# facebookresearch/vggsfm

Measured on NVIDIA H100. Metric: BA iterations/sec, higher is better.
Workload: dtype f64

## Files before the change

vggsfm_b200/_lib.py:

```python
from __future__ import annotations

import ctypes
import os

_HERE = os.path.dirname(os.path.abspath(__file__))
LIB_PATH = os.path.join(_HERE, "libvggsfm_b200.so")

EXPORTS = [
    "vgg_last_error", "vgg_version",
    "vgg_ba_default_options", "vgg_ba_dims", "vgg_ba_workspace_bytes", "vgg_ba_camrec_len",
    "vgg_ba_build_blocks", "vgg_ba_schur", "vgg_cholesky_lower", "vgg_ba_solve",
    "vgg_ba_reduced_system_doubles", "vgg_ba_fabric_doubles", "vgg_ba_solve_fabric",
    "vgg_pose_default_options", "vgg_pose_refinement", "vgg_pnp_workspace_bytes", "vgg_absolute_pose_estimation", "vgg_syrk_ozaki_workspace_bytes", "vgg_syrk_ozaki",
    "vgg_tri_workspace_bytes", "vgg_triangulate_tracks", "vgg_triangulate_by_pair", "vgg_filter_points3d",
    "vgg_project_points", "vgg_normalize_tracks", "vgg_undistort_simple_radial",
    "vgg_corr_pyramid_bytes", "vgg_corr_build_pyramid", "vgg_corr_sample", "vgg_sample_features4d",
    "vgg_corr_tc_supported", "vgg_corr_tc_bytes", "vgg_corr_tc_build", "vgg_corr_tc_sample",
    "vgg_twoview_workspace_bytes", "vgg_estimate_fundamental", "vgg_relative_pose_from_fundamental",
    "vgg_fundamental_inliers", "vgg_msac_fundamental_workspace_bytes", "vgg_estimate_fundamental_msac",
    "vgg_depth_sparse_samples", "vgg_depth_median", "vgg_depth_ransac_workspace_bytes", "vgg_depth_ransac_max_chunk",
    "vgg_depth_ransac_begin", "vgg_depth_ransac_chunk", "vgg_depth_ransac_finish", "vgg_depth_tile_pixels",
    "vgg_depth_apply", "vgg_depth_unproject",
]


DEV_EXPORTS = ["vgg_dev_blocks_timing", "vgg_dev_blocks_last_ms", "vgg_dev_chol128_probe", "vgg_dev_syrk_f64", "vgg_dev_syrk_f64_band", "vgg_dev_syrk_ozaki_band", "vgg_dev_trsv_probe", "vgg_dev_cholesky_band",
               "vgg_dev_last_band_hint", "vgg_dev_msac_trace"]


class BAProblem(ctypes.Structure):
    _fields_ = [
        ("S", ctypes.c_int32), ("N", ctypes.c_int32),
        ("camera_model", ctypes.c_int32), ("intr_mode", ctypes.c_int32),
        ("uv", ctypes.c_void_p), ("mask", ctypes.c_void_p),
        ("param_const", ctypes.c_void_p), ("point_const", ctypes.c_void_p),
        ("poses", ctypes.c_void_p), ("intr", ctypes.c_void_p), ("points", ctypes.c_void_p),
    ]


class BAOptions(ctypes.Structure):
    _fields_ = [
        ("max_num_iterations", ctypes.c_int32),
        ("max_num_consecutive_invalid_steps", ctypes.c_int32),
        ("jacobi_scaling", ctypes.c_int32),
        ("reserved", ctypes.c_int32),
        ("function_tolerance", ctypes.c_double),
        ("gradient_tolerance", ctypes.c_double),
        ("parameter_tolerance", ctypes.c_double),
        ("initial_trust_region_radius", ctypes.c_double),
        ("max_trust_region_radius", ctypes.c_double),
        ("min_trust_region_radius", ctypes.c_double),
        ("min_relative_decrease", ctypes.c_double),
        ("min_lm_diagonal", ctypes.c_double),
        ("max_lm_diagonal", ctypes.c_double),
    ]


class BASummary(ctypes.Structure):
    _fields_ = [
        ("iterations", ctypes.c_int32), ("successful", ctypes.c_int32),
        ("termination", ctypes.c_int32), ("reserved", ctypes.c_int32),
        ("initial_cost", ctypes.c_double), ("final_cost", ctypes.c_double),
        ("final_radius", ctypes.c_double), ("device_ms", ctypes.c_double),
        ("kernel_launches", ctypes.c_int64),
    ]


class BAFabric(ctypes.Structure):
    _fields_ = [("ar_local", ctypes.c_void_p), ("ar_multicast", ctypes.c_void_p), ("ar_doubles", ctypes.c_size_t),
                ("world", ctypes.c_int32), ("rank", ctypes.c_int32), ("peer_base", ctypes.c_void_p * 8),
                ("total_doubles", ctypes.c_size_t)]


class PoseOptions(ctypes.Structure):
    _fields_ = [
        ("max_num_iterations", ctypes.c_int32),
        ("max_num_consecutive_invalid_steps", ctypes.c_int32),
        ("min_inliers", ctypes.c_int32),
        ("reserved", ctypes.c_int32),
        ("function_tolerance", ctypes.c_double),
        ("gradient_tolerance", ctypes.c_double),
        ("parameter_tolerance", ctypes.c_double),
        ("initial_trust_region_radius", ctypes.c_double),
        ("max_trust_region_radius", ctypes.c_double),
        ("min_trust_region_radius", ctypes.c_double),
        ("min_relative_decrease", ctypes.c_double),
        ("min_lm_diagonal", ctypes.c_double),
        ("max_lm_diagonal", ctypes.c_double),
        ("loss_function_scale", ctypes.c_double),
        ("max_reproj_error", ctypes.c_double),
    ]


ALLREDUCE_FN = ctypes.CFUNCTYPE(ctypes.c_int, ctypes.c_void_p, ctypes.c_void_p, ctypes.c_size_t,
                                ctypes.c_int, ctypes.c_void_p)

_lib = None


class NativeLibraryMissing(RuntimeError):
    pass


def lib() -> ctypes.CDLL:
    global _lib
    if _lib is not None:
        return _lib
    if not os.path.exists(LIB_PATH):
        raise NativeLibraryMissing(
            f"{LIB_PATH} not found: build it with `python -c 'import __graft_entry__ as g; g.build()'` "
            "or `make`. vggsfm_b200 has no CPU/PyTorch fallback.")
    L = ctypes.CDLL(LIB_PATH, mode=ctypes.RTLD_GLOBAL)
    L.vgg_last_error.restype = ctypes.c_char_p
    L.vgg_version.restype = ctypes.c_int
    L.vgg_ba_default_options.argtypes = [ctypes.POINTER(BAOptions)]
    L.vgg_ba_default_options.restype = None
    L.vgg_ba_dims.argtypes = [ctypes.c_int, ctypes.c_int, ctypes.POINTER(ctypes.c_int), ctypes.POINTER(ctypes.c_int)]
    L.vgg_ba_workspace_bytes.argtypes = [ctypes.c_int, ctypes.c_int, ctypes.c_int, ctypes.c_int,
                                         ctypes.POINTER(ctypes.c_size_t)]
    L.vgg_ba_camrec_len.argtypes = [ctypes.c_int, ctypes.c_int]
    L.vgg_ba_build_blocks.argtypes = [ctypes.POINTER(BAProblem)] + [ctypes.c_void_p] * 6 + [ctypes.c_int, ctypes.c_void_p]
    L.vgg_ba_schur.argtypes = ([ctypes.POINTER(BAProblem)] + [ctypes.c_void_p] * 6 +
                               [ctypes.c_double] * 3 + [ctypes.c_void_p, ctypes.c_size_t, ctypes.c_void_p,
                                                        ctypes.c_void_p, ctypes.POINTER(ctypes.c_int), ctypes.c_void_p])
    L.vgg_ba_solve.argtypes = [ctypes.POINTER(BAProblem), ctypes.POINTER(BAOptions), ctypes.c_void_p, ctypes.c_size_t,
                               ALLREDUCE_FN, ctypes.c_void_p, ctypes.POINTER(BASummary), ctypes.c_void_p,
                               ctypes.c_void_p]
    vp, ci, cd, cs = ctypes.c_void_p, ctypes.c_int, ctypes.c_double, ctypes.c_size_t
    L.vgg_ba_reduced_system_doubles.argtypes = [ci, ci, ci, ctypes.POINTER(cs)]
    L.vgg_ba_fabric_doubles.argtypes = [ci, ci, ci, ctypes.POINTER(cs)]
    L.vgg_ba_solve_fabric.argtypes = [ctypes.POINTER(BAProblem), ctypes.POINTER(BAOptions), vp, cs, ALLREDUCE_FN, vp,
                                      ctypes.POINTER(BAFabric), ctypes.POINTER(BASummary), vp, vp]
    L.vgg_pose_default_options.argtypes = [ctypes.POINTER(PoseOptions)]
    L.vgg_pose_default_options.restype = None
    L.vgg_pose_refinement.argtypes = [ci, ci, ci, vp, vp, vp, vp, vp, vp, ctypes.POINTER(PoseOptions), vp, vp, vp, vp]
    L.vgg_pnp_workspace_bytes.argtypes = [ci, ci, ctypes.POINTER(cs)]
    L.vgg_absolute_pose_estimation.argtypes = [ci, ci, ci, vp, vp, vp, vp, vp, vp, ci, ci, cd, vp, vp, vp, vp, vp, cs, vp]
    L.vgg_syrk_ozaki_workspace_bytes.argtypes = [ci, ci, ci, ctypes.POINTER(cs)]
    L.vgg_dev_blocks_timing.argtypes = [ci]
    L.vgg_dev_blocks_last_ms.argtypes = [ctypes.POINTER(cd)]
    L.vgg_dev_chol128_probe.argtypes = [ci, vp, vp, vp]
    L.vgg_dev_syrk_f64.argtypes = [ci, ci, vp, vp, vp]
    L.vgg_dev_syrk_f64_band.argtypes = L.vgg_dev_syrk_f64.argtypes + [vp, ci]
    L.vgg_dev_trsv_probe.argtypes = [ci, ci, vp, vp, cs, vp, vp]
    L.vgg_dev_last_band_hint.argtypes = [vp, vp, vp, vp, vp]
    L.vgg_syrk_ozaki.argtypes = [ci, ci, vp, vp, ci, vp, cs, vp]
    L.vgg_dev_syrk_ozaki_band.argtypes = L.vgg_syrk_ozaki.argtypes + [vp, ci]
    L.vgg_cholesky_lower.argtypes = [ci, ci, vp, vp, cs, ctypes.POINTER(ci), vp]
    L.vgg_dev_cholesky_band.argtypes = L.vgg_cholesky_lower.argtypes + [vp, ci, ci]
    L.vgg_tri_workspace_bytes.argtypes = [ci, ci, ci, ci, ctypes.POINTER(cs)]
    L.vgg_triangulate_tracks.argtypes = [ci, ci, vp, vp, vp, vp, vp, ci, ci, cd, cd, vp, vp, vp, vp, cs, vp]
    L.vgg_triangulate_by_pair.argtypes = [ci, ci, vp, vp, vp, vp, vp, vp, cs, vp]
    L.vgg_filter_points3d.argtypes = [ci, ci, vp, vp, ci, vp, vp, vp, cd, cd, ci, cd, vp, vp, vp, cs, vp]
    L.vgg_project_points.argtypes = [ci, ci, vp, vp, vp, vp, vp, vp, vp]
    L.vgg_normalize_tracks.argtypes = [ci, ci, vp, vp, vp, ci, vp, vp]
    L.vgg_undistort_simple_radial.argtypes = [ci, ci, vp, vp, ci, cd, cd, vp, ctypes.POINTER(ci), vp, cs, vp]
    L.vgg_corr_pyramid_bytes.argtypes = [ci, ci, ci, ci, ci, ci, ctypes.POINTER(cs), ctypes.POINTER(cs)]
    L.vgg_corr_build_pyramid.argtypes = [ci, ci, ci, ci, ci, vp, ci, vp, vp, vp]
    L.vgg_sample_features4d.argtypes = [ci, ci, ci, ci, ci, vp, vp, vp, vp]
    L.vgg_corr_sample.argtypes = [ci, ci, ci, ci, ci, ci, ci, vp, ci, vp, vp, ci, vp, vp]
    L.vgg_corr_tc_supported.argtypes = [ci, ci, ci, ci, ci]
    L.vgg_corr_tc_bytes.argtypes = [ci, ci, ci, ci, ci, ci, ctypes.POINTER(cs), ctypes.POINTER(cs)]
    L.vgg_corr_tc_build.argtypes = [ci, ci, ci, ci, ci, vp, vp, vp]
    L.vgg_corr_tc_sample.argtypes = [ci, ci, ci, ci, ci, ci, ci, vp, vp, vp, vp, vp, vp]
    L.vgg_twoview_workspace_bytes.argtypes = [ci, ci, ci, ci, ctypes.POINTER(cs)]
    L.vgg_estimate_fundamental.argtypes = [ci, ci, vp, vp, ci, vp, vp, ci, ci, cd, ci, ci, vp, vp, vp, vp, vp, cs, vp]
    L.vgg_fundamental_inliers.argtypes = [ci, ci, vp, vp, ci, vp, cd, ci, vp, vp]
    L.vgg_relative_pose_from_fundamental.argtypes = [ci, ci, vp, vp, ci, vp, cd, cd, vp, vp, vp, vp]
    cu64 = ctypes.c_ulonglong
    L.vgg_msac_fundamental_workspace_bytes.argtypes = [ci, ci, ci, ci, ctypes.POINTER(cs)]
    L.vgg_estimate_fundamental_msac.argtypes = [ci, ci, vp, vp, ci, vp, cd, ci, ci, cu64, vp, vp, vp, vp, vp, cs, vp]
    L.vgg_dev_msac_trace.argtypes = [ci, ci, ci, ci, vp, ci, vp, vp, vp]
    i64 = ctypes.c_int64
    L.vgg_depth_sparse_samples.argtypes = [ci, vp, vp, cd, cd, vp, vp, vp, vp, vp, vp, vp]
    L.vgg_depth_median.argtypes = [ci, vp, vp, cd, vp, vp]
    L.vgg_depth_ransac_workspace_bytes.argtypes = [ci, ctypes.POINTER(cs)]
    L.vgg_depth_ransac_max_chunk.argtypes = []
    L.vgg_depth_ransac_begin.argtypes = [ci, ci, vp, cs, vp]
    L.vgg_depth_ransac_chunk.argtypes = [ci, vp, vp, vp, vp, ci, vp, ci, vp, vp, vp, cs, vp]
    L.vgg_depth_ransac_finish.argtypes = [ci, vp, vp, vp, vp, vp, vp, vp, vp, vp, vp, cs, vp]
    L.vgg_depth_tile_pixels.argtypes = []
    L.vgg_depth_apply.argtypes = [ci, i64, vp, vp, vp, vp, vp, vp, vp, vp]
    L.vgg_depth_unproject.argtypes = [ci, i64, vp, vp, vp, vp, vp, vp, vp, vp, vp, vp, vp]
    _lib = L
    return L


def check(rc: int, what: str) -> None:
    if rc != 0:
        raise RuntimeError(f"{what} failed (rc={rc}): {lib().vgg_last_error().decode(errors='replace')}")
```

vggsfm_b200/csrc/chol.cu:

```cuda
#include <stdlib.h>
#include <algorithm>
#include <map>
#include <vector>
#include <tuple>
#include "common.cuh"

namespace vgg {

constexpr int CB = 128;
constexpr int CLD = 132;
constexpr int C_RPC = 16;
constexpr int C_RPC_MAX = 32;
constexpr int CT = 64;
constexpr int C_THREADS = 256;

__device__ __forceinline__ double fast_rsqrt(double p) {
  double r;
  asm("rsqrt.approx.ftz.f64 %0, %1;" : "=d"(r) : "d"(p));
  const double hp = 0.5 * p;
  r = r * fma(-hp * r, r, 1.5);
  r = r * fma(-hp * r, r, 1.5);
  return r;
}
constexpr double CHOL_PMIN = 2.2250738585072014e-308;

template <bool PROBE>
__device__ __forceinline__ int cta_chol128(double* Ls, double* dinv, int* fail_sm, int tid, int xr,
                                           long long* prof = nullptr) {
  const int lane = tid & 31, warp = tid >> 5;
  __shared__ __align__(16) double Lh[64];
  if (tid == 0) *fail_sm = 0;
  __syncthreads();
  auto tri_row = [](int e) { return (e >= 1) + (e >= 3) + (e >= 6) + (e >= 10) + (e >= 15) + (e >= 21) + (e >= 28); };
  const int pi0 = tri_row(lane), pj0 = lane - pi0 * (pi0 + 1) / 2;
  const int e1 = lane < 4 ? lane + 32 : 35;
  const int pi1 = tri_row(e1), pj1 = e1 - pi1 * (pi1 + 1) / 2;
  long long pacc[6] = {0, 0, 0, 0, 0, 0}, plast = 0;
  const bool ptid = PROBE && (tid == 0 || tid == 32);
  if (ptid) plast = clock64();
#define CHOL_MARK(ph)                         \
  if (ptid) {                                 \
    const long long t_ = clock64();           \
    pacc[ph] += t_ - plast;                   \
    plast = t_;                               \
  }
  auto leaf = [&](int c0) {
    double a[8];
    const int r = c0 + (lane & 7);
#pragma unroll
    for (int c = 0; c < 8; c += 2) {
      const double2 v = *reinterpret_cast<const double2*>(Ls + r * CLD + c0 + c);
      a[c] = v.x;
      a[c + 1] = v.y;
    }
    int fail = 0;
    double mydinv = 1.0;
#pragma unroll
    for (int j = 0; j < 8; j += 2) {
      const double A = __shfl_sync(0xffffffffu, a[j], j);
      const double B = __shfl_sync(0xffffffffu, a[j], j + 1);
      const double C = __shfl_sync(0xffffffffu, a[j + 1], j + 1);
      const double AC = A * C;
      const double det = fma(-B, B, AC);
      double ia = fast_rsqrt(A);
      const double rdet = fast_rsqrt(det);
      double ib = (A * ia) * rdet;
      double d11 = (det * rdet) * ia;
      double l10 = B * ia;
      const bool good = A >= CHOL_PMIN && det >= CHOL_PMIN && AC < 1e280 && AC > 1e-280;
      if (!good) {
        if (!(A >= CHOL_PMIN)) {
          if (fail == 0) fail = c0 + j + 1;
          ia = 1.0;
          l10 = B;
        }
        const double p1 = fma(-l10, l10, C);
        if (!(p1 >= CHOL_PMIN)) {
          if (fail == 0) fail = c0 + j + 2;
          ib = 1.0;
        } else {
          ib = rsqrt(p1);
        }
        d11 = p1 * ib;
      }
      const double x0 = a[j] * ia;
      const double x1 = lane == j + 1 ? d11 : fma(-x0, l10, a[j + 1]) * ib;
      a[j] = x0;
      a[j + 1] = x1;
      if (lane == j) {
        dinv[c0 + j] = ia;
        dinv[c0 + j + 1] = ib;
        mydinv = ia;
      }
      if (lane == j + 1) mydinv = ib;
#pragma unroll
      for (int c = j + 2; c < 8; ++c) {
        const double l0 = __shfl_sync(0xffffffffu, x0, c);
        const double l1 = __shfl_sync(0xffffffffu, x1, c);
        if (lane >= c) a[c] = fma(-x1, l1, fma(-x0, l0, a[c]));
      }
    }
    if (lane < 8) {
#pragma unroll
      for (int c = 0; c < 8; ++c) Ls[r * CLD + c0 + c] = (c <= lane) ? a[c] : 0.0;
#pragma unroll
      for (int c = 0; c < 8; ++c) Lh[lane * 8 + c] = (c < lane) ? a[c] * mydinv : 0.0;
    }
    if (lane == 0 && fail && *fail_sm == 0) *fail_sm = fail;
  };
  auto row_update = [&](int r, int c0, int jb, int js, int jend) {
    double li[8];
#pragma unroll
    for (int k = 0; k < 8; k += 2) {
      const double2 v = *reinterpret_cast<const double2*>(Ls + r * CLD + c0 + k);
      li[k] = v.x;
      li[k + 1] = v.y;
    }
    int j = jb;
    for (; j + js <= jend; j += 2 * js) {
      const double* l0 = Ls + j * CLD + c0;
      const double* l1 = Ls + (j + js) * CLD + c0;
      double s0 = Ls[r * CLD + j], s1 = Ls[r * CLD + j + js];
#pragma unroll
      for (int k = 0; k < 8; k += 2) {
        const double2 u = *reinterpret_cast<const double2*>(l0 + k);
        const double2 w = *reinterpret_cast<const double2*>(l1 + k);
        s0 = fma(-li[k], u.x, s0);
        s1 = fma(-li[k], w.x, s1);
        s0 = fma(-li[k + 1], u.y, s0);
        s1 = fma(-li[k + 1], w.y, s1);
      }
      Ls[r * CLD + j] = s0;
      Ls[r * CLD + j + js] = s1;
    }
    if (j <= jend) {
      const double* l0 = Ls + j * CLD + c0;
      double s0 = Ls[r * CLD + j];
#pragma unroll
      for (int k = 0; k < 8; k += 2) {
        const double2 u = *reinterpret_cast<const double2*>(l0 + k);
        s0 = fma(-li[k], u.x, s0);
        s0 = fma(-li[k + 1], u.y, s0);
      }
      Ls[r * CLD + j] = s0;
    }
  };
  if (warp == 0) leaf(0);
  __syncthreads();
  CHOL_MARK(0)
  for (int sp = 0; sp < CB / 32; ++sp) {
    const int c32 = sp * 32;
    for (int mp = 0; mp < 4; ++mp) {
      const int c0 = c32 + mp * 8;
      {
        const int r = c0 + 8 + tid;
        if (r < CB + xr) {
          double x[8];
#pragma unroll
          for (int c = 0; c < 8; c += 2) {
            const double2 v = *reinterpret_cast<const double2*>(Ls + r * CLD + c0 + c);
            x[c] = v.x;
            x[c + 1] = v.y;
          }
#pragma unroll
          for (int m = 0; m < 8; ++m) x[m] *= dinv[c0 + m];
#pragma unroll
          for (int m = 1; m < 8; ++m) {
#pragma unroll
            for (int k = 0; k < m; ++k) x[m] = fma(-x[k], Lh[m * 8 + k], x[m]);
          }
#pragma unroll
          for (int c = 0; c < 8; c += 2) *reinterpret_cast<double2*>(Ls + r * CLD + c0 + c) = make_double2(x[c], x[c + 1]);
        }
      }
      __syncthreads();
      CHOL_MARK(1)
      if (mp < 3) {
        const int n0 = c0 + 8;
        if (warp == 0) {
          {
            const double* ri = Ls + (n0 + pi0) * CLD + c0;
            const double* rj = Ls + (n0 + pj0) * CLD + c0;
            const double* ri1 = Ls + (n0 + pi1) * CLD + c0;
            const double* rj1 = Ls + (n0 + pj1) * CLD + c0;
            double s0 = Ls[(n0 + pi0) * CLD + n0 + pj0], s1 = 0.0;
            double u0 = Ls[(n0 + pi1) * CLD + n0 + pj1], u1 = 0.0;
#pragma unroll
            for (int k = 0; k < 8; k += 4) {
              const double2 a0 = *reinterpret_cast<const double2*>(ri + k), a1 = *reinterpret_cast<const double2*>(ri + k + 2);
              const double2 b0 = *reinterpret_cast<const double2*>(rj + k), b1 = *reinterpret_cast<const double2*>(rj + k + 2);
              const double2 c0v = *reinterpret_cast<const double2*>(ri1 + k), c1v = *reinterpret_cast<const double2*>(ri1 + k + 2);
              const double2 d0 = *reinterpret_cast<const double2*>(rj1 + k), d1 = *reinterpret_cast<const double2*>(rj1 + k + 2);
              s0 = fma(-a0.x, b0.x, s0);
              s1 = fma(-a0.y, b0.y, s1);
              u0 = fma(-c0v.x, d0.x, u0);
              u1 = fma(-c0v.y, d0.y, u1);
              s0 = fma(-a1.x, b1.x, s0);
              s1 = fma(-a1.y, b1.y, s1);
              u0 = fma(-c1v.x, d1.x, u0);
              u1 = fma(-c1v.y, d1.y, u1);
            }
            Ls[(n0 + pi0) * CLD + n0 + pj0] = s0 + s1;
            if (lane < 4) Ls[(n0 + pi1) * CLD + n0 + pj1] = u0 + u1;
          }
          __syncwarp();
          leaf(n0);
        } else {
          const int t = tid - 32;
          for (int rr = t >> 1; n0 + rr < CB + xr; rr += 112) {
            const int r = n0 + rr, half = t & 1;
            const int jend = min(r, c32 + 31);
            if (r < n0 + 8) continue;
            row_update(r, c0, n0 + half, 2, jend);
          }
        }
        CHOL_MARK(2)
        __syncthreads();
        CHOL_MARK(3)
      }
    }
    const int t0 = c32 + 32;
    const int nrb = (CB - t0) / 32;
    if (nrb > 0) {
      const int ntile = nrb * (nrb + 1);
      const int nxt = xr ? (CB - t0) / 16 : 0;
      const int rend = CB + xr;
      const int g = lane >> 2, q = lane & 3;
      bool leaf_pending = warp == 0;
      for (int t = warp == 0 ? 0 : warp; t < ntile + nxt; t += (warp == 0 ? ntile + nxt : C_THREADS / 32 - 1)) {
        int R0, C0, nrow16 = 2;
        if (t < ntile) {
          int rb = 0, cb = t;
          while (cb >= 2 * rb + 2) { cb -= 2 * rb + 2; ++rb; }
          R0 = t0 + rb * 32;
          C0 = t0 + cb * 16;
        } else {
          R0 = CB;
          C0 = t0 + (t - ntile) * 16;
          nrow16 = (xr + 15) / 16;
        }
        double c[2][2][4];
#pragma unroll
        for (int i = 0; i < 2; ++i)
#pragma unroll
          for (int j = 0; j < 2; ++j) c[i][j][0] = c[i][j][1] = c[i][j][2] = c[i][j][3] = 0.0;
#pragma unroll
        for (int kk = c32; kk < c32 + 32; kk += 16) {
          double a[2][8], b[2][4];
#pragma unroll
          for (int j = 0; j < 2; ++j)
#pragma unroll
            for (int e = 0; e < 4; ++e) b[j][e] = Ls[(C0 + j * 8 + g) * CLD + kk + q + 4 * e];
#pragma unroll
          for (int i = 0; i < 2; ++i) {
            if (i < nrow16) {
#pragma unroll
              for (int e = 0; e < 8; ++e) {
                const int r = R0 + i * 16 + g + 8 * (e & 1);
                a[i][e] = r < rend ? Ls[r * CLD + kk + q + 4 * (e >> 1)] : 0.0;
              }
#pragma unroll
              for (int j = 0; j < 2; ++j) dmma_m16n8k16(c[i][j], a[i], b[j]);
            }
          }
        }
#pragma unroll
        for (int i = 0; i < 2; ++i) {
          if (i >= nrow16) continue;
#pragma unroll
          for (int h = 0; h < 2; ++h) {
            const int r = R0 + i * 16 + g + 8 * h;
            if (r >= rend) continue;
#pragma unroll
            for (int j = 0; j < 2; ++j) {
              const int col = C0 + j * 8 + 2 * q;
              if (col > r) continue;
              double* pp = Ls + r * CLD + col;
              if (col + 1 <= r) {
                double2 v = *reinterpret_cast<double2*>(pp);
                v.x -= c[i][j][2 * h];
                v.y -= c[i][j][2 * h + 1];
                *reinterpret_cast<double2*>(pp) = v;
              } else {
                *pp -= c[i][j][2 * h];
              }
            }
          }
        }
        if (leaf_pending) {
          __syncwarp();
          leaf(t0);
          leaf_pending = false;
        }
      }
      CHOL_MARK(4)
      __syncthreads();
      CHOL_MARK(5)
    }
  }
#undef CHOL_MARK
  if (ptid) {
#pragma unroll
    for (int i = 0; i < 6; ++i) prof[(tid == 32 ? 6 : 0) + i] = pacc[i];
  }
  return *fail_sm;
}

__global__ void __launch_bounds__(C_THREADS, 1) chol128_probe_kernel(const double* __restrict__ A, double* __restrict__ L,
                                                                      long long* __restrict__ prof, int reps, int xr) {
  extern __shared__ __align__(16) double cp_smem[];
  __shared__ double dinv[CB];
  __shared__ int fail_sm;
  const int tid = threadIdx.x;
  long long total = 0;
  for (int rep = 0; rep < reps; ++rep) {
    for (int e = tid; e < CB * CB; e += C_THREADS) cp_smem[(e >> 7) * CLD + (e & 127)] = A[e];
    for (int e = tid; e < xr * CB; e += C_THREADS)
      cp_smem[(CB + (e >> 7)) * CLD + (e & 127)] = A[(CB - xr + (e >> 7)) * CB + (e & 127)];
    __syncthreads();
    const long long t0 = clock64();
    cta_chol128<true>(cp_smem, dinv, &fail_sm, tid, xr, prof);
    __syncthreads();
    total = clock64() - t0;
  }
  if (tid == 0) prof[12] = total;
  for (int e = tid; e < CB * CB; e += C_THREADS) L[e] = ((e & 127) <= (e >> 7)) ? cp_smem[(e >> 7) * CLD + (e & 127)] : 0.0;
}

constexpr int CHOL_SPIN_LIMIT = 1 << 22;
constexpr int CHOL_INFO_STALLED = 0x7fffffff;

__global__ void __launch_bounds__(C_THREADS, 1) chol_panel_kernel(int n, int lda, int k0, double* __restrict__ A,
                                                                   double* __restrict__ Ldiag ,
                                                                   int* __restrict__ info, int* __restrict__ flags,
                                                                   int fuse, int band_end, int arrow_lo, int xr) {
  extern __shared__ __align__(16) double cp_smem[];
  double* Ls = cp_smem;
  double* Ts = cp_smem + CB * CLD;
  __shared__ double dinv[CB];
  __shared__ int fail_sm;
  const int tid = threadIdx.x, lane = tid & 31, warp = tid >> 5;
  const int nb = min(CB, n - k0);
  const bool solver = blockIdx.x > 0;
  const int band_hi = min(band_end, n);
  const int chunks1r = (max(0, band_hi - (k0 + CB)) + xr - 1) / xr;
  const int cidx = (int)blockIdx.x - 1;
  const int r0 = cidx < chunks1r ? k0 + CB + cidx * xr : arrow_lo + (cidx - chunks1r) * xr;
  const int nrows = solver ? min(xr, (cidx < chunks1r ? band_hi : n) - r0) : 0;
  for (int e = tid; e < CB * (CB / 2); e += C_THREADS) {
    const int i = e >> 6, j = (e & 63) * 2;
    if (i < nb && j + 1 < nb) {
      cp_async16(Ls + i * CLD + j, A + (size_t)(k0 + i) * lda + k0 + j);
    } else if (i < nb) {
      *reinterpret_cast<double2*>(Ls + i * CLD + j) = make_double2(j < nb ? A[(size_t)(k0 + i) * lda + k0 + j] : 0.0, 0.0);
    } else {
      *reinterpret_cast<double2*>(Ls + i * CLD + j) = make_double2(j == i ? 1.0 : 0.0, j + 1 == i ? 1.0 : 0.0);
    }
  }
  for (int e = tid; e < xr * (CB / 2); e += C_THREADS) {
    const int r = e >> 6, j = (e & 63) * 2;
    if (r < nrows) cp_async16(Ts + r * CLD + j, A + (size_t)(r0 + r) * lda + k0 + j);
    else *reinterpret_cast<double2*>(Ts + r * CLD + j) = make_double2(0.0, 0.0);
  }
  cp_async_commit();
  cp_async_wait<0>();
  __syncthreads();
  const int fail = cta_chol128<false>(Ls, dinv, &fail_sm, tid, xr);
  if (fail && blockIdx.x == 0 && tid == 0) atomicCAS(info, 0, k0 + fail);
  if (!solver) {
    const bool alone = gridDim.x == 1;
    double* dst = Ldiag + (size_t)(k0 / CB) * CB * CB;
    for (int e = tid; e < CB * CB; e += C_THREADS) {
      const int i = e >> 7, j = e & 127;
      if (i < nb && j < nb) {
        if (j > i) A[(size_t)(k0 + i) * lda + k0 + j] = Ls[j * CLD + i];
        else if (alone) A[(size_t)(k0 + i) * lda + k0 + j] = Ls[i * CLD + j];
        else dst[e] = Ls[i * CLD + j];
      }
    }
    if (k0 > 0) {
      const double* src = Ldiag + (size_t)(k0 / CB - 1) * CB * CB;
      double* blk = A + (size_t)(k0 - CB) * lda + (k0 - CB);
      for (int e0 = tid; e0 < CB * CB; e0 += 8 * C_THREADS) {
        double v[8];
#pragma unroll
        for (int u = 0; u < 8; ++u) {
          const int e = e0 + u * C_THREADS;
          v[u] = ((e & 127) <= (e >> 7)) ? __ldcg(src + e) : 0.0;
        }
#pragma unroll
        for (int u = 0; u < 8; ++u) {
          const int e = e0 + u * C_THREADS;
          const int i = e >> 7, j = e & 127;
          if (j <= i) blk[(size_t)i * lda + j] = v[u];
        }
      }
    }
    return;
  }
  for (int e = tid; e < nrows * CB; e += C_THREADS) {
    const int r = e >> 7, c = e & 127;
    if (c < nb) A[(size_t)(r0 + r) * lda + k0 + c] = Ts[r * CLD + c];
  }
  for (int e = tid; e < nrows * CB; e += C_THREADS) {
    const int c = e / nrows, r = e - c * nrows;
    if (c < nb) A[(size_t)(k0 + c) * lda + r0 + r] = Ts[r * CLD + c];
  }
  if (!fuse) return;

  const int t0 = k0 + CB;
  const bool p_active = band_end > t0 || arrow_lo == t0;
  const int nprod = p_active ? min((CB + xr - 1) / xr, (int)gridDim.x - 1) : 0;
  if (nprod == 0) return;
  int* flag = flags + k0 / CB;
  __threadfence();
  __syncthreads();
  if (tid == 0) {
    if ((int)blockIdx.x <= nprod) atomicAdd(flag, 1);
    int spins = 0, seen;
    do {
      asm volatile("ld.acquire.gpu.global.s32 %0, [%1];" : "=r"(seen) : "l"(flag) : "memory");
    } while (seen < nprod && ++spins < CHOL_SPIN_LIMIT);
    if (seen < nprod) atomicCAS(info, 0, CHOL_INFO_STALLED);
  }
  __syncthreads();
#pragma unroll
  for (int half = 0; half < 2; ++half) {
    for (int e = tid; e < CB * 16; e += C_THREADS) {
      const int row = e >> 4, ch = (e & 15) * 4 + half * 64;
      double* dst = Ls + row * CLD + ch;
      if (t0 + row < n) {
        const double* src = A + (size_t)(t0 + row) * lda + k0 + ch;
        cp_async16(dst, src);
        cp_async16(dst + 2, src + 2);
      } else {
        *reinterpret_cast<double2*>(dst) = make_double2(0.0, 0.0);
        *reinterpret_cast<double2*>(dst + 2) = make_double2(0.0, 0.0);
      }
    }
    cp_async_commit();
  }
  {
    const int g = lane >> 2, q = lane & 3;
    const int nrow16 = (xr + 15) / 16;
    double c[2][2][4];
#pragma unroll
    for (int i = 0; i < 2; ++i)
#pragma unroll
      for (int j = 0; j < 2; ++j) c[i][j][0] = c[i][j][1] = c[i][j][2] = c[i][j][3] = 0.0;
#pragma unroll
    for (int half = 0; half < 2; ++half) {
      if (half == 0) cp_async_wait<1>();
      else cp_async_wait<0>();
      __syncthreads();
#pragma unroll 2
      for (int kk = half * 64; kk < half * 64 + 64; kk += 16) {
        double a[2][8], b[2][4];
#pragma unroll
        for (int j = 0; j < 2; ++j)
#pragma unroll
          for (int e = 0; e < 4; ++e) b[j][e] = Ls[(warp * 16 + j * 8 + g) * CLD + kk + q + 4 * e];
#pragma unroll
        for (int i = 0; i < 2; ++i) {
          if (i < nrow16) {
#pragma unroll
            for (int e = 0; e < 8; ++e) {
              const int r = i * 16 + g + 8 * (e & 1);
              a[i][e] = r < xr ? Ts[r * CLD + kk + q + 4 * (e >> 1)] : 0.0;
            }
#pragma unroll
            for (int j = 0; j < 2; ++j) dmma_m16n8k16(c[i][j], a[i], b[j]);
          }
        }
      }
    }
#pragma unroll
    for (int i = 0; i < 2; ++i) {
#pragma unroll
      for (int h = 0; h < 2; ++h) {
        const int rr = i * 16 + g + 8 * h;
        if (i >= nrow16 || rr >= nrows) continue;
        const int r = r0 + rr;
#pragma unroll
        for (int j = 0; j < 2; ++j) {
          const int col = t0 + warp * 16 + j * 8 + 2 * q;
          double* p = A + (size_t)r * lda + col;
          if (col <= r) atomicAdd(p, -c[i][j][2 * h]);
          if (col + 1 <= r) atomicAdd(p + 1, -c[i][j][2 * h + 1]);
        }
      }
    }
  }
}

constexpr int CUD = 68;
enum { CU_ALL = 0, CU_NEXT = 1, CU_REST = 2 };
__global__ void __launch_bounds__(C_THREADS, 2) chol_update_kernel(int n, int lda, int k0, int t0, int mode,
                                                                    double* __restrict__ A, int band_end, int arrow_lo,
                                                                    int all_red) {
  extern __shared__ __align__(16) double cu_smem[];
  double* As = cu_smem;
  double* Bs = cu_smem + CT * CUD;
  int bi, bj;
  {
    const int t = blockIdx.x;
    if (mode == CU_NEXT) {
      const int T = (max(0, min(band_end, n) - t0) + 63) / 64 + (band_end >= n ? 0 : (n - arrow_lo + 63) / 64);
      if (t < T - 2) { bi = 2 + t; bj = 2; }
      else { bi = 3 + (t - (T - 2)); bj = 3; }
    } else {
      bi = (int)((sqrtf(8.0f * (float)t + 1.0f) - 1.0f) * 0.5f);
      while ((bi + 1) * (bi + 2) / 2 <= t) ++bi;
      while (bi * (bi + 1) / 2 > t) --bi;
      bj = t - bi * (bi + 1) / 2;
      const int skip = mode == CU_REST ? 4 : 0;
      bi += skip;
      bj += skip;
    }
  }
  const bool diag = bi == bj;
  const int tid = threadIdx.x, lane = tid & 31, warp = tid >> 5;
  const int T1v = band_end >= n ? (1 << 30) : (band_end - t0) / 64;
  auto vrow = [&](int v) { return v < T1v ? t0 + v * 64 : arrow_lo + (v - T1v) * 64; };
  const int ri = vrow(bi), rj = vrow(bj);
  const double* bs = diag ? As : Bs;
  const int wm = warp / 4, wn = warp % 4;
  const int g = lane >> 2, q = lane & 3;
  double c[2][2][4];
#pragma unroll
  for (int i = 0; i < 2; ++i)
#pragma unroll
    for (int j = 0; j < 2; ++j) c[i][j][0] = c[i][j][1] = c[i][j][2] = c[i][j][3] = 0.0;
  const double* arow = As + (wm * 32 + g) * CUD + q;
  const double* brow = bs + (wn * 16 + g) * CUD + q;
#pragma unroll 1
  for (int half = 0; half < 2; ++half) {
    if (half) __syncthreads();
    for (int e = tid; e < 2 * CT * 16; e += C_THREADS) {
      const int row = e >> 4, ch = (e & 15) * 4;
      const bool isA = row < CT;
      if (!isA && diag) continue;
      const int grow = isA ? ri + row : rj + (row - CT);
      double* dst = (isA ? As + row * CUD : Bs + (row - CT) * CUD) + ch;
      if (grow < n) {
        const double* src = A + (size_t)grow * lda + k0 + half * 64 + ch;
        cp_async16(dst, src);
        cp_async16(dst + 2, src + 2);
      } else {
        *reinterpret_cast<double2*>(dst) = make_double2(0.0, 0.0);
        *reinterpret_cast<double2*>(dst + 2) = make_double2(0.0, 0.0);
      }
    }
    cp_async_commit();
    cp_async_wait<0>();
    __syncthreads();
#pragma unroll 2
    for (int kk = 0; kk < 64; kk += 16) {
      double a[2][8], b[2][4];
#pragma unroll
      for (int i = 0; i < 2; ++i)
#pragma unroll
        for (int e = 0; e < 8; ++e) a[i][e] = arow[(i * 16 + 8 * (e & 1)) * CUD + kk + 4 * (e >> 1)];
#pragma unroll
      for (int j = 0; j < 2; ++j)
#pragma unroll
        for (int e = 0; e < 4; ++e) b[j][e] = brow[j * 8 * CUD + kk + 4 * e];
#pragma unroll
      for (int i = 0; i < 2; ++i)
#pragma unroll
        for (int j = 0; j < 2; ++j) dmma_m16n8k16(c[i][j], a[i], b[j]);
    }
  }
  const bool red = all_red || mode == CU_NEXT || (mode == CU_REST && bj < 6);
#pragma unroll
  for (int i = 0; i < 2; ++i) {
#pragma unroll
    for (int h = 0; h < 2; ++h) {
      const int r = ri + wm * 32 + i * 16 + g + 8 * h;
      if (r >= n) continue;
#pragma unroll
      for (int j = 0; j < 2; ++j) {
        const int col = rj + wn * 16 + j * 8 + 2 * q;
        if (col > r) continue;
        double* p = A + (size_t)r * lda + col;
        const double v0 = c[i][j][2 * h], v1 = c[i][j][2 * h + 1];
        if (red) {
          atomicAdd(p, -v0);
          if (col + 1 <= r) atomicAdd(p + 1, -v1);
        } else if (col + 1 <= r) {
          double2 v = *reinterpret_cast<double2*>(p);
          v.x -= v0;
          v.y -= v1;
          *reinterpret_cast<double2*>(p) = v;
        } else {
          *p -= v0;
        }
      }
    }
  }
}


size_t chol_workspace_doubles(int n) {
  const int nblk = (n + CB - 1) / CB;
  return (size_t)nblk * CB * CB + (size_t)(nblk + 1) / 2 + 1;
}

namespace {

struct CholStreams {
  cudaStream_t side_lo = nullptr, side_mid = nullptr, cap = nullptr;
  cudaEvent_t ev_col = nullptr, ev_upd[2] = {nullptr, nullptr}, ev_bulk[3] = {nullptr, nullptr, nullptr};
  bool ready = false;
};

int chol_streams(CholStreams** out) {
  static thread_local CholStreams s;
  if (!s.ready) {
    int lo = 0, hi = 0;
    VGG_CUDA_CHECK(cudaDeviceGetStreamPriorityRange(&lo, &hi));
    VGG_CUDA_CHECK(cudaStreamCreateWithPriority(&s.side_lo, cudaStreamNonBlocking, lo));
    VGG_CUDA_CHECK(cudaStreamCreateWithPriority(&s.side_mid, cudaStreamNonBlocking, (lo + hi) / 2));
    VGG_CUDA_CHECK(cudaStreamCreateWithPriority(&s.cap, cudaStreamNonBlocking, hi));
    VGG_CUDA_CHECK(cudaEventCreateWithFlags(&s.ev_col, cudaEventDisableTiming));
    VGG_CUDA_CHECK(cudaEventCreateWithFlags(&s.ev_upd[0], cudaEventDisableTiming));
    VGG_CUDA_CHECK(cudaEventCreateWithFlags(&s.ev_upd[1], cudaEventDisableTiming));
    for (int i = 0; i < 3; ++i) VGG_CUDA_CHECK(cudaEventCreateWithFlags(&s.ev_bulk[i], cudaEventDisableTiming));
    s.ready = true;
  }
  *out = &s;
  return VGG_OK;
}

int chol_sms() {
  static const int v = [] {
    int dev = 0, sms = 0;
    if (cudaGetDevice(&dev) != cudaSuccess || cudaDeviceGetAttribute(&sms, cudaDevAttrMultiProcessorCount, dev) != cudaSuccess)
      sms = 0;
    return sms > 0 ? sms : 132;
  }();
  return v;
}

int chol_set_attrs() {
  static bool done = false;
  if (done) return VGG_OK;
  VGG_CUDA_CHECK(cudaFuncSetAttribute(chol_panel_kernel, cudaFuncAttributeMaxDynamicSharedMemorySize,
                                      (int)(sizeof(double) * (CB + C_RPC_MAX) * CLD)));
  VGG_CUDA_CHECK(cudaFuncSetAttribute(chol_update_kernel, cudaFuncAttributeMaxDynamicSharedMemorySize,
                                      (int)(sizeof(double) * 2 * CT * CUD)));
  done = true;
  return VGG_OK;
}

int chol_panel_rows(int below1, int below2, int* chunks) {
  const int sms = chol_sms();
  int xr = C_RPC;
  for (;; xr += 4) {
    *chunks = (below1 + xr - 1) / xr + (below2 + xr - 1) / xr;
    if (1 + *chunks <= sms || xr >= C_RPC_MAX) return xr;
  }
}

int chol_enqueue(int n, int lda, double* A, double* Ldiag, int* info, int* flags, const std::vector<int>& end_blk,
                 int arrow_blk, cudaStream_t st, CholStreams* cs, bool lookahead) {
  const int nblk = (n + CB - 1) / CB;
  const size_t smem_u = sizeof(double) * 2 * CT * CUD;
  const bool banded = lookahead && (int)end_blk.size() >= nblk && arrow_blk > 0;
  auto band_rows = [&](int b, int* band_end, int* arrow_lo) {
    if (!banded) {
      *band_end = *arrow_lo = n;
      return;
    }
    *band_end = std::min(n, end_blk[b] * CB);
    *arrow_lo = std::min(n, std::max(arrow_blk * CB, *band_end));
    if (*band_end >= n || *arrow_lo <= *band_end) *band_end = *arrow_lo = n;
  };
  auto panel = [&](int b) -> int {
    const int k0 = b * CB;
    int band_end, arrow_lo, chunks;
    band_rows(b, &band_end, &arrow_lo);
    const int below1 = std::max(0, std::min(band_end, n) - (k0 + CB));
    const int below2 = band_end >= n ? 0 : n - arrow_lo;
    const int xr = chol_panel_rows(below1, below2, &chunks);
    const size_t smem_p = sizeof(double) * (CB + xr) * CLD;
    const int fuse = lookahead ? 1 : 0;
    chol_panel_kernel<<<1 + chunks, C_THREADS, smem_p, st>>>(n, lda, k0, A, Ldiag, info, flags, fuse, band_end, arrow_lo, xr);
    VGG_LAUNCH_CHECK();
    return VGG_OK;
  };
  int rc;
  if ((rc = panel(0))) return rc;
  if (!lookahead) {
    for (int b = 0; b + 1 < nblk; ++b) {
      const int k0 = b * CB, t0 = k0 + CB;
      const int T = (n - t0 + CT - 1) / CT;
      chol_update_kernel<<<T * (T + 1) / 2, C_THREADS, smem_u, st>>>(n, lda, k0, t0, CU_ALL, A, n, n, 0);
      VGG_LAUNCH_CHECK();
      if ((rc = panel(b + 1))) return rc;
    }
    return VGG_OK;
  }
  bool have_u1[2] = {false, false}, have_u2[3] = {false, false, false};
  for (int b = 0; b + 1 < nblk; ++b) {
    const int k0 = b * CB, t0 = k0 + CB;
    int band_end, arrow_lo;
    band_rows(b, &band_end, &arrow_lo);
    const int T = (std::max(0, std::min(band_end, n) - t0) + CT - 1) / CT + (band_end >= n ? 0 : (n - arrow_lo + CT - 1) / CT);
    const int all_red = band_end >= n ? 0 : 1;
    const int n_u1 = T > 2 ? (T - 2) + (T > 3 ? T - 3 : 0) : 0;
    const int n_u2 = T > 4 ? (T - 4) * (T - 3) / 2 : 0;
    have_u1[b & 1] = false;
    have_u2[b % 3] = false;
    if (n_u1 > 0) {
      VGG_CUDA_CHECK(cudaEventRecord(cs->ev_col, st));
      VGG_CUDA_CHECK(cudaStreamWaitEvent(cs->side_mid, cs->ev_col, 0));
      if (b >= 2 && have_u2[(b - 2) % 3]) VGG_CUDA_CHECK(cudaStreamWaitEvent(cs->side_mid, cs->ev_bulk[(b - 2) % 3], 0));
      chol_update_kernel<<<n_u1, C_THREADS, smem_u, cs->side_mid>>>(n, lda, k0, t0, CU_NEXT, A, band_end, arrow_lo, all_red);
      VGG_LAUNCH_CHECK();
      VGG_CUDA_CHECK(cudaEventRecord(cs->ev_upd[b & 1], cs->side_mid));
      have_u1[b & 1] = true;
      if (n_u2 > 0) {
        VGG_CUDA_CHECK(cudaStreamWaitEvent(cs->side_lo, cs->ev_col, 0));
        chol_update_kernel<<<n_u2, C_THREADS, smem_u, cs->side_lo>>>(n, lda, k0, t0, CU_REST, A, band_end, arrow_lo, all_red);
        VGG_LAUNCH_CHECK();
        VGG_CUDA_CHECK(cudaEventRecord(cs->ev_bulk[b % 3], cs->side_lo));
        have_u2[b % 3] = true;
      }
    }
    if (b >= 1 && have_u1[(b - 1) & 1]) VGG_CUDA_CHECK(cudaStreamWaitEvent(st, cs->ev_upd[(b - 1) & 1], 0));
    if (b >= 2 && have_u2[(b - 2) % 3]) VGG_CUDA_CHECK(cudaStreamWaitEvent(st, cs->ev_bulk[(b - 2) % 3], 0));
    if ((rc = panel(b + 1))) return rc;
  }
  for (int i = 0; i < 2; ++i)
    if (have_u1[i]) VGG_CUDA_CHECK(cudaStreamWaitEvent(st, cs->ev_upd[i], 0));
  for (int i = 0; i < 3; ++i)
    if (have_u2[i]) VGG_CUDA_CHECK(cudaStreamWaitEvent(st, cs->ev_bulk[i], 0));
  return VGG_OK;
}

}

int chol_lower_inplace(int n, int lda, double* A, double* Ldiag, int* info, const std::vector<int>& end_blk,
                       int arrow_blk, cudaStream_t st) {
  VGG_REQUIRE((lda % 2) == 0, "lda must be even");
  int rc;
  if ((rc = chol_set_attrs())) return rc;
  VGG_CUDA_CHECK(cudaMemsetAsync(info, 0, sizeof(int), st));
  const int nblk0 = (n + CB - 1) / CB;
  int* flags = reinterpret_cast<int*>(Ldiag + (size_t)nblk0 * CB * CB);
  VGG_CUDA_CHECK(cudaMemsetAsync(flags, 0, sizeof(int) * (size_t)nblk0, st));
  static const bool use_graph = [] { const char* e = getenv("VGG_CHOL_GRAPH"); return !(e && e[0] == '0'); }();
  const int nblk = (n + CB - 1) / CB;
  CholStreams* cs = nullptr;
  if ((rc = chol_streams(&cs))) return rc;
  if (nblk < 3 || !use_graph) return chol_enqueue(n, lda, A, Ldiag, info, flags, end_blk, arrow_blk, st, cs, nblk >= 3);
  typedef std::tuple<double*, int, int, int*, double*, unsigned long long> Key;
  static thread_local std::map<Key, cudaGraphExec_t> cache;
  unsigned long long band_hash = (unsigned long long)arrow_blk;
  for (int v : end_blk) band_hash = band_hash * 1000003ull + (unsigned long long)(v + 1);
  const Key key(A, n, lda, info, Ldiag, band_hash);
  auto it = cache.find(key);
  if (it == cache.end()) {
    const long long launches_before = g_launch_count;
    cudaGraph_t graph = nullptr;
    VGG_CUDA_CHECK(cudaStreamBeginCapture(cs->cap, cudaStreamCaptureModeThreadLocal));
    rc = chol_enqueue(n, lda, A, Ldiag, info, flags, end_blk, arrow_blk, cs->cap, cs, true);
    const cudaError_t ce = cudaStreamEndCapture(cs->cap, &graph);
    g_launch_count = launches_before;
    if (rc) {
      if (graph) cudaGraphDestroy(graph);
      return rc;
    }
    VGG_CUDA_CHECK(ce);
    cudaGraphExec_t exec = nullptr;
    VGG_CUDA_CHECK(cudaGraphInstantiate(&exec, graph, 0));
    cudaGraphDestroy(graph);
    if (cache.size() > 8) {
      for (auto& kv : cache) cudaGraphExecDestroy(kv.second);
      cache.clear();
    }
    it = cache.emplace(key, exec).first;
  }
  VGG_CUDA_CHECK(cudaGraphLaunch(it->second, st));
  g_launch_count += 1 + 3 * (nblk - 1);
  return VGG_OK;
}

}

extern "C" int vgg_dev_chol128_probe(int reps, const double* A_host, double* L_host, long long* prof13_host) {
  using namespace vgg;
  VGG_REQUIRE(A_host && L_host && prof13_host && reps > 0, "chol128 probe: bad arguments");
  double *dA = nullptr, *dL = nullptr;
  long long* dP = nullptr;
  VGG_CUDA_CHECK(cudaMalloc(&dA, sizeof(double) * CB * CB));
  VGG_CUDA_CHECK(cudaMalloc(&dL, sizeof(double) * CB * CB));
  VGG_CUDA_CHECK(cudaMalloc(&dP, sizeof(long long) * 13));
  VGG_CUDA_CHECK(cudaMemcpy(dA, A_host, sizeof(double) * CB * CB, cudaMemcpyHostToDevice));
  VGG_CUDA_CHECK(cudaMemset(dP, 0, sizeof(long long) * 13));
  const int smem = (int)(sizeof(double) * (CB + C_RPC) * CLD);
  VGG_CUDA_CHECK(cudaFuncSetAttribute(chol128_probe_kernel, cudaFuncAttributeMaxDynamicSharedMemorySize, smem));
  chol128_probe_kernel<<<1, C_THREADS, smem>>>(dA, dL, dP, reps, C_RPC);
  VGG_LAUNCH_CHECK();
  VGG_CUDA_CHECK(cudaDeviceSynchronize());
  VGG_CUDA_CHECK(cudaMemcpy(L_host, dL, sizeof(double) * CB * CB, cudaMemcpyDeviceToHost));
  VGG_CUDA_CHECK(cudaMemcpy(prof13_host, dP, sizeof(long long) * 13, cudaMemcpyDeviceToHost));
  cudaFree(dA);
  cudaFree(dL);
  cudaFree(dP);
  return VGG_OK;
}
```

vggsfm_b200/csrc/dev_probes.h:

```cpp
#pragma once
#ifdef __cplusplus
extern "C" {
#endif
int vgg_dev_blocks_timing(int enable);
int vgg_dev_blocks_last_ms(double* ms);
int vgg_dev_chol128_probe(int reps, const double* A_host, double* L_host, long long* prof13_host);
int vgg_dev_syrk_f64(int Kpad, int Dpad, const double* Zt, double* Cmat, void* stream);
int vgg_dev_syrk_f64_band(int Kpad, int Dpad, const double* Zt, double* Cmat, void* stream, const int* ranges_host,
                          int count);
int vgg_dev_syrk_ozaki_band(int Kpad, int Dpad, const double* Zt, double* Cmat, int slices, void* workspace,
                            size_t ws_bytes, void* stream, const int* ranges_host, int count);
int vgg_dev_trsv_probe(int n, int lda, const double* A_dev, const double* y_dev, size_t y_stride, double* x_dev,
                       long long* stamps_host);
int vgg_dev_last_band_hint(int* meta_host, int* rb_range, int* end_blk, int* kb_rows, int* fg_tracks);
int vgg_dev_cholesky_band(int n, int lda, double* A, void* workspace, size_t ws_bytes, int* info_host, void* stream,
                          const int* end_blk_host, int count, int arrow_blk);
int vgg_dev_msac_trace(int B, int N, int max_iterations, int min_iterations, const void* workspace, int cap,
                       int32_t* lo_runs_host, int32_t* win_trial_host, int32_t* lo_trials_host);

#ifdef __cplusplus
}
#endif
```

Measured before the change: 338.4.

## Replace graph-captured multi-stream blocked Cholesky with a persistent cooperative kernel

Blocked Cholesky used to run as a CUDA graph of panel and update kernels spread over several streams linked by events. It now runs as a single cooperative persistent kernel. Panel CTAs synchronise through named barriers and global step counters with acquire loads, and a separate barrier group handles the trailing updates. The aim is to remove per-step launch and event latency and let panel and update work overlap at finer grain. The cost is spin-wait dependencies, a fixed row-chunk size, and atomicAdd-based trailing updates that can change numerical order. Optional globaltimer stamps are added for per-step profiling.

```diff
diff --git a/vggsfm_b200/_lib.py b/vggsfm_b200/_lib.py
--- a/vggsfm_b200/_lib.py
+++ b/vggsfm_b200/_lib.py
@@ -24,7 +24,7 @@
 ]
 
 
-DEV_EXPORTS = ["vgg_dev_blocks_timing", "vgg_dev_blocks_last_ms", "vgg_dev_chol128_probe", "vgg_dev_syrk_f64", "vgg_dev_syrk_f64_band", "vgg_dev_syrk_ozaki_band", "vgg_dev_trsv_probe", "vgg_dev_cholesky_band",
+DEV_EXPORTS = ["vgg_dev_blocks_timing", "vgg_dev_blocks_last_ms", "vgg_dev_chol128_probe", "vgg_dev_chol_stamps", "vgg_dev_chol_last_stamps", "vgg_dev_syrk_f64", "vgg_dev_syrk_f64_band", "vgg_dev_syrk_ozaki_band", "vgg_dev_trsv_probe", "vgg_dev_cholesky_band",
                "vgg_dev_last_band_hint", "vgg_dev_msac_trace"]
 
 
@@ -140,6 +140,8 @@
     L.vgg_dev_blocks_timing.argtypes = [ci]
     L.vgg_dev_blocks_last_ms.argtypes = [ctypes.POINTER(cd)]
     L.vgg_dev_chol128_probe.argtypes = [ci, vp, vp, vp]
+    L.vgg_dev_chol_stamps.argtypes = [ci]
+    L.vgg_dev_chol_last_stamps.argtypes = [vp, ci, ctypes.POINTER(ci)]
     L.vgg_dev_syrk_f64.argtypes = [ci, ci, vp, vp, vp]
     L.vgg_dev_syrk_f64_band.argtypes = L.vgg_dev_syrk_f64.argtypes + [vp, ci]
     L.vgg_dev_trsv_probe.argtypes = [ci, ci, vp, vp, cs, vp, vp]
diff --git a/vggsfm_b200/csrc/chol.cu b/vggsfm_b200/csrc/chol.cu
--- a/vggsfm_b200/csrc/chol.cu
+++ b/vggsfm_b200/csrc/chol.cu
@@ -1,9 +1,7 @@
-#include <stdlib.h>
 #include <algorithm>
-#include <map>
 #include <vector>
-#include <tuple>
 #include "common.cuh"
+#include "dev_probes.h"
 
 namespace vgg {
 
@@ -24,13 +22,16 @@
 }
 constexpr double CHOL_PMIN = 2.2250738585072014e-308;
 
+__device__ __forceinline__ void panel_sync() { asm volatile("bar.sync 1, 256;" ::: "memory"); }
+__device__ __forceinline__ void group_sync(int id) { asm volatile("bar.sync %0, 256;" ::"r"(id) : "memory"); }
+
 template <bool PROBE>
 __device__ __forceinline__ int cta_chol128(double* Ls, double* dinv, int* fail_sm, int tid, int xr,
                                            long long* prof = nullptr) {
   const int lane = tid & 31, warp = tid >> 5;
   __shared__ __align__(16) double Lh[64];
   if (tid == 0) *fail_sm = 0;
-  __syncthreads();
+  panel_sync();
   auto tri_row = [](int e) { return (e >= 1) + (e >= 3) + (e >= 6) + (e >= 10) + (e >= 15) + (e >= 21) + (e >= 28); };
   const int pi0 = tri_row(lane), pj0 = lane - pi0 * (pi0 + 1) / 2;
   const int e1 = lane < 4 ? lane + 32 : 35;
@@ -146,7 +147,7 @@
     }
   };
   if (warp == 0) leaf(0);
-  __syncthreads();
+  panel_sync();
   CHOL_MARK(0)
   for (int sp = 0; sp < CB / 32; ++sp) {
     const int c32 = sp * 32;
@@ -173,7 +174,7 @@
           for (int c = 0; c < 8; c += 2) *reinterpret_cast<double2*>(Ls + r * CLD + c0 + c) = make_double2(x[c], x[c + 1]);
         }
       }
-      __syncthreads();
+      panel_sync();
       CHOL_MARK(1)
       if (mp < 3) {
         const int n0 = c0 + 8;
@@ -215,7 +216,7 @@
           }
         }
         CHOL_MARK(2)
-        __syncthreads();
+        panel_sync();
         CHOL_MARK(3)
       }
     }
@@ -294,7 +295,7 @@
         }
       }
       CHOL_MARK(4)
-      __syncthreads();
+      panel_sync();
       CHOL_MARK(5)
     }
   }
@@ -327,58 +328,157 @@
   for (int e = tid; e < CB * CB; e += C_THREADS) L[e] = ((e & 127) <= (e >> 7)) ? cp_smem[(e >> 7) * CLD + (e & 127)] : 0.0;
 }
 
+constexpr int CHOL_MAX_BLK = 1024;
+struct CholArgs {
+  int n, lda, nblk, arrow_blk, sms, banded;
+  int xr_fixed;
+  int panel_ctas;
+  double* A;
+  double* Ldiag;
+  int* info;
+  int* ctr;
+  long long* stamps;
+  unsigned short end_blk[CHOL_MAX_BLK];
+};
+struct StepGeo {
+  int k0, band_end, arrow_lo, xr, chunks1r, chunks, T, T1v;
+};
+__host__ __device__ inline StepGeo step_geo(const CholArgs& a, int b) {
+  StepGeo g;
+  const int n = a.n;
+  g.k0 = b * CB;
+  g.band_end = g.arrow_lo = n;
+  if (a.banded) {
+    g.band_end = min(n, (int)a.end_blk[b] * CB);
+    g.arrow_lo = min(n, max(a.arrow_blk * CB, g.band_end));
+    if (g.band_end >= n || g.arrow_lo <= g.band_end) g.band_end = g.arrow_lo = n;
+  }
+  const int band_hi = min(g.band_end, n);
+  const int below1 = max(0, band_hi - (g.k0 + CB));
+  const int below2 = g.band_end >= n ? 0 : n - g.arrow_lo;
+  for (g.xr = a.xr_fixed > 0 ? a.xr_fixed : C_RPC;; g.xr += 4) {
+    g.chunks1r = (below1 + g.xr - 1) / g.xr;
+    g.chunks = g.chunks1r + (below2 + g.xr - 1) / g.xr;
+    if (a.xr_fixed > 0 || 1 + g.chunks <= a.sms || g.xr >= C_RPC_MAX) break;
+  }
+  const int t0 = g.k0 + CB;
+  g.T = (max(0, band_hi - t0) + CT - 1) / CT + (g.band_end >= n ? 0 : (n - g.arrow_lo + CT - 1) / CT);
+  g.T1v = g.band_end >= n ? (1 << 30) : (g.band_end - t0) / CT;
+  return g;
+}
+__host__ __device__ inline int tile_row(const StepGeo& g, int v) {
+  return v < g.T1v ? g.k0 + CB + v * CT : g.arrow_lo + (v - g.T1v) * CT;
+}
+__host__ __device__ inline int step_tiles(const StepGeo& g) { return g.T > 2 ? (g.T - 2) * (g.T - 1) / 2 : 0; }
+__device__ inline int step_first_tile_col(const StepGeo& g, int n, int c) {
+  const int r = c * CB, t0 = g.k0 + CB;
+  if (r >= t0 && r < min(g.band_end, n)) return (r - t0) / CT;
+  if (g.band_end < n && r >= g.arrow_lo && r < n) return g.T1v + (r - g.arrow_lo) / CT;
+  return -1;
+}
+__device__ inline int step_tiles_in_col(const StepGeo& g, int n, int c) {
+  const int bj0 = step_first_tile_col(g, n, c);
+  if (bj0 < 0) return 0;
+  int cnt = 0;
+  for (int bj = max(bj0, 2); bj <= bj0 + 1 && bj < g.T; ++bj) cnt += g.T - bj;
+  return cnt;
+}
+
+__device__ inline int step_chunk_at(const StepGeo& g, int n, int r, int* next) {
+  const int band_hi = min(g.band_end, n), t0 = g.k0 + CB;
+  if (r >= t0 && r < band_hi) {
+    const int c = (r - t0) / g.xr;
+    *next = min(band_hi, t0 + (c + 1) * g.xr);
+    return 1 + c;
+  }
+  if (g.band_end < n && r >= g.arrow_lo) {
+    const int c = (r - g.arrow_lo) / g.xr;
+    *next = min(n, g.arrow_lo + (c + 1) * g.xr);
+    return 1 + g.chunks1r + c;
+  }
+  *next = g.band_end < n && r < g.arrow_lo && r >= band_hi ? g.arrow_lo : n;
+  return 0;
+}
+
 constexpr int CHOL_SPIN_LIMIT = 1 << 22;
 constexpr int CHOL_INFO_STALLED = 0x7fffffff;
-
-__global__ void __launch_bounds__(C_THREADS, 1) chol_panel_kernel(int n, int lda, int k0, double* __restrict__ A,
-                                                                   double* __restrict__ Ldiag ,
-                                                                   int* __restrict__ info, int* __restrict__ flags,
-                                                                   int fuse, int band_end, int arrow_lo, int xr) {
-  extern __shared__ __align__(16) double cp_smem[];
-  double* Ls = cp_smem;
-  double* Ts = cp_smem + CB * CLD;
-  __shared__ double dinv[CB];
-  __shared__ int fail_sm;
-  const int tid = threadIdx.x, lane = tid & 31, warp = tid >> 5;
+__device__ __forceinline__ int ld_acquire(const int* p) {
+  int v;
+  asm volatile("ld.acquire.gpu.global.s32 %0, [%1];" : "=r"(v) : "l"(p) : "memory");
+  return v;
+}
+__device__ inline void chol_wait(const int* p, int shift, int mask, int target, int* info, bool nap) {
+  int spins = 0, seen;
+  while (((seen = ld_acquire(p)) >> shift & mask) < target) {
+    if (++spins >= CHOL_SPIN_LIMIT || ((spins & 255) == 0 && ld_acquire(info) == CHOL_INFO_STALLED)) {
+      atomicCAS(info, 0, CHOL_INFO_STALLED);
+      return;
+    }
+    if (nap) __nanosleep(200);
+  }
+}
+__device__ __forceinline__ long long globaltimer() {
+  long long t;
+  asm volatile("mov.u64 %0, %%globaltimer;" : "=l"(t));
+  return t;
+}
+
+struct PanelJob {
+  int n, lda, k0, band_end, arrow_lo, xr, chunks, v;
+  int* prev_ctr;
+  int prev_chunks;
+};
+__device__ __forceinline__ void panel_step(const PanelJob& j, double* __restrict__ A, double* __restrict__ Ldiag,
+                                           int* __restrict__ info, double* Ls, double* dinv, int* fail_sm, int tid,
+                                           int* step_ctr, long long* stamp) {
+  double* Ts = Ls + CB * CLD;
+  const int lane = tid & 31, warp = tid >> 5;
+  const int n = j.n, lda = j.lda, k0 = j.k0, xr = j.xr;
+  if (stamp && tid == 0) stamp[1] = globaltimer();
   const int nb = min(CB, n - k0);
-  const bool solver = blockIdx.x > 0;
-  const int band_hi = min(band_end, n);
+  const bool solver = j.v > 0;
+  const int band_hi = min(j.band_end, n);
   const int chunks1r = (max(0, band_hi - (k0 + CB)) + xr - 1) / xr;
-  const int cidx = (int)blockIdx.x - 1;
-  const int r0 = cidx < chunks1r ? k0 + CB + cidx * xr : arrow_lo + (cidx - chunks1r) * xr;
+  const int cidx = j.v - 1;
+  const int r0 = cidx < chunks1r ? k0 + CB + cidx * xr : j.arrow_lo + (cidx - chunks1r) * xr;
   const int nrows = solver ? min(xr, (cidx < chunks1r ? band_hi : n) - r0) : 0;
   for (int e = tid; e < CB * (CB / 2); e += C_THREADS) {
-    const int i = e >> 6, j = (e & 63) * 2;
-    if (i < nb && j + 1 < nb) {
-      cp_async16(Ls + i * CLD + j, A + (size_t)(k0 + i) * lda + k0 + j);
+    const int i = e >> 6, jc = (e & 63) * 2;
+    if (i < nb && jc + 1 < nb) {
+      cp_async16(Ls + i * CLD + jc, A + (size_t)(k0 + i) * lda + k0 + jc);
     } else if (i < nb) {
-      *reinterpret_cast<double2*>(Ls + i * CLD + j) = make_double2(j < nb ? A[(size_t)(k0 + i) * lda + k0 + j] : 0.0, 0.0);
+      *reinterpret_cast<double2*>(Ls + i * CLD + jc) = make_double2(jc < nb ? A[(size_t)(k0 + i) * lda + k0 + jc] : 0.0, 0.0);
     } else {
-      *reinterpret_cast<double2*>(Ls + i * CLD + j) = make_double2(j == i ? 1.0 : 0.0, j + 1 == i ? 1.0 : 0.0);
+      *reinterpret_cast<double2*>(Ls + i * CLD + jc) = make_double2(jc == i ? 1.0 : 0.0, jc + 1 == i ? 1.0 : 0.0);
     }
   }
   for (int e = tid; e < xr * (CB / 2); e += C_THREADS) {
-    const int r = e >> 6, j = (e & 63) * 2;
-    if (r < nrows) cp_async16(Ts + r * CLD + j, A + (size_t)(r0 + r) * lda + k0 + j);
-    else *reinterpret_cast<double2*>(Ts + r * CLD + j) = make_double2(0.0, 0.0);
+    const int r = e >> 6, jc = (e & 63) * 2;
+    if (r < nrows) cp_async16(Ts + r * CLD + jc, A + (size_t)(r0 + r) * lda + k0 + jc);
+    else *reinterpret_cast<double2*>(Ts + r * CLD + jc) = make_double2(0.0, 0.0);
   }
   cp_async_commit();
   cp_async_wait<0>();
-  __syncthreads();
-  const int fail = cta_chol128<false>(Ls, dinv, &fail_sm, tid, xr);
-  if (fail && blockIdx.x == 0 && tid == 0) atomicCAS(info, 0, k0 + fail);
+  panel_sync();
+  const int fail = cta_chol128<false>(Ls, dinv, fail_sm, tid, xr);
+  if (stamp && tid == 0) stamp[2] = globaltimer();
+  if (fail && j.v == 0 && tid == 0) atomicCAS(info, 0, k0 + fail);
   if (!solver) {
-    const bool alone = gridDim.x == 1;
+    const bool alone = j.chunks == 0;
     double* dst = Ldiag + (size_t)(k0 / CB) * CB * CB;
     for (int e = tid; e < CB * CB; e += C_THREADS) {
-      const int i = e >> 7, j = e & 127;
-      if (i < nb && j < nb) {
-        if (j > i) A[(size_t)(k0 + i) * lda + k0 + j] = Ls[j * CLD + i];
-        else if (alone) A[(size_t)(k0 + i) * lda + k0 + j] = Ls[i * CLD + j];
-        else dst[e] = Ls[i * CLD + j];
+      const int i = e >> 7, jc = e & 127;
+      if (i < nb && jc < nb) {
+        if (jc > i) A[(size_t)(k0 + i) * lda + k0 + jc] = Ls[jc * CLD + i];
+        else if (alone) A[(size_t)(k0 + i) * lda + k0 + jc] = Ls[i * CLD + jc];
+        else dst[e] = Ls[i * CLD + jc];
       }
     }
     if (k0 > 0) {
+      if (j.prev_ctr) {
+        if (tid == 0) chol_wait(j.prev_ctr, 0, 0xffff, j.prev_chunks, info, false);
+        panel_sync();
+      }
       const double* src = Ldiag + (size_t)(k0 / CB - 1) * CB * CB;
       double* blk = A + (size_t)(k0 - CB) * lda + (k0 - CB);
       for (int e0 = tid; e0 < CB * CB; e0 += 8 * C_THREADS) {
@@ -391,11 +491,12 @@
 #pragma unroll
         for (int u = 0; u < 8; ++u) {
           const int e = e0 + u * C_THREADS;
-          const int i = e >> 7, j = e & 127;
-          if (j <= i) blk[(size_t)i * lda + j] = v[u];
-        }
-      }
-    }
+          const int i = e >> 7, jc = e & 127;
+          if (jc <= i) blk[(size_t)i * lda + jc] = v[u];
+        }
+      }
+    }
+    if (stamp && tid == 0) stamp[3] = globaltimer();
     return;
   }
   for (int e = tid; e < nrows * CB; e += C_THREADS) {
@@ -406,31 +507,134 @@
     const int c = e / nrows, r = e - c * nrows;
     if (c < nb) A[(size_t)(k0 + c) * lda + r0 + r] = Ts[r * CLD + c];
   }
-  if (!fuse) return;
+  if (!step_ctr) return;
 
   const int t0 = k0 + CB;
-  const bool p_active = band_end > t0 || arrow_lo == t0;
-  const int nprod = p_active ? min((CB + xr - 1) / xr, (int)gridDim.x - 1) : 0;
-  if (nprod == 0) return;
-  int* flag = flags + k0 / CB;
+  const bool p_active = j.band_end > t0 || j.arrow_lo == t0;
+  const int nprod = p_active ? min((CB + xr - 1) / xr, j.chunks) : 0;
   __threadfence();
-  __syncthreads();
+  panel_sync();
+  if (nprod > 0) {
+    if (tid == 0) {
+      if (j.v <= nprod) atomicAdd(step_ctr, 1 << 16);
+      chol_wait(step_ctr, 16, 0xffff, nprod, info, false);
+    }
+    panel_sync();
+#pragma unroll
+    for (int half = 0; half < 2; ++half) {
+      for (int e = tid; e < CB * 16; e += C_THREADS) {
+        const int row = e >> 4, ch = (e & 15) * 4 + half * 64;
+        double* dst = Ls + row * CLD + ch;
+        if (t0 + row < n) {
+          const double* src = A + (size_t)(t0 + row) * lda + k0 + ch;
+          cp_async16(dst, src);
+          cp_async16(dst + 2, src + 2);
+        } else {
+          *reinterpret_cast<double2*>(dst) = make_double2(0.0, 0.0);
+          *reinterpret_cast<double2*>(dst + 2) = make_double2(0.0, 0.0);
+        }
+      }
+      cp_async_commit();
+    }
+    const int g = lane >> 2, q = lane & 3;
+    const int nrow16 = (xr + 15) / 16;
+    double c[2][2][4];
+#pragma unroll
+    for (int i = 0; i < 2; ++i)
+#pragma unroll
+      for (int jj = 0; jj < 2; ++jj) c[i][jj][0] = c[i][jj][1] = c[i][jj][2] = c[i][jj][3] = 0.0;
+#pragma unroll
+    for (int half = 0; half < 2; ++half) {
+      if (half == 0) cp_async_wait<1>();
+      else cp_async_wait<0>();
+      panel_sync();
+#pragma unroll 2
+      for (int kk = half * 64; kk < half * 64 + 64; kk += 16) {
+        double a[2][8], b[2][4];
+#pragma unroll
+        for (int jj = 0; jj < 2; ++jj)
+#pragma unroll
+          for (int e = 0; e < 4; ++e) b[jj][e] = Ls[(warp * 16 + jj * 8 + g) * CLD + kk + q + 4 * e];
+#pragma unroll
+        for (int i = 0; i < 2; ++i) {
+          if (i < nrow16) {
+#pragma unroll
+            for (int e = 0; e < 8; ++e) {
+              const int r = i * 16 + g + 8 * (e & 1);
+              a[i][e] = r < xr ? Ts[r * CLD + kk + q + 4 * (e >> 1)] : 0.0;
+            }
+#pragma unroll
+            for (int jj = 0; jj < 2; ++jj) dmma_m16n8k16(c[i][jj], a[i], b[jj]);
+          }
+        }
+      }
+    }
+#pragma unroll
+    for (int i = 0; i < 2; ++i) {
+#pragma unroll
+      for (int h = 0; h < 2; ++h) {
+        const int rr = i * 16 + g + 8 * h;
+        if (i >= nrow16 || rr >= nrows) continue;
+        const int r = r0 + rr;
+#pragma unroll
+        for (int jj = 0; jj < 2; ++jj) {
+          const int col = t0 + warp * 16 + jj * 8 + 2 * q;
+          double* p = A + (size_t)r * lda + col;
+          if (col <= r) atomicAdd(p, -c[i][jj][2 * h]);
+          if (col + 1 <= r) atomicAdd(p + 1, -c[i][jj][2 * h + 1]);
+        }
+      }
+    }
+    __threadfence();
+    panel_sync();
+  }
   if (tid == 0) {
-    if ((int)blockIdx.x <= nprod) atomicAdd(flag, 1);
-    int spins = 0, seen;
-    do {
-      asm volatile("ld.acquire.gpu.global.s32 %0, [%1];" : "=r"(seen) : "l"(flag) : "memory");
-    } while (seen < nprod && ++spins < CHOL_SPIN_LIMIT);
-    if (seen < nprod) atomicCAS(info, 0, CHOL_INFO_STALLED);
-  }
-  __syncthreads();
-#pragma unroll
-  for (int half = 0; half < 2; ++half) {
-    for (int e = tid; e < CB * 16; e += C_THREADS) {
-      const int row = e >> 4, ch = (e & 15) * 4 + half * 64;
-      double* dst = Ls + row * CLD + ch;
-      if (t0 + row < n) {
-        const double* src = A + (size_t)(t0 + row) * lda + k0 + ch;
+    __threadfence();
+    atomicAdd(step_ctr, 1);
+    if (stamp) stamp[3] = globaltimer();
+  }
+}
+
+__global__ void __launch_bounds__(C_THREADS, 1) chol_panel_kernel(int n, int lda, int k0, double* __restrict__ A,
+                                                                   double* __restrict__ Ldiag, int* __restrict__ info,
+                                                                   int xr, int chunks) {
+  extern __shared__ __align__(16) double cp_smem[];
+  __shared__ double dinv[CB];
+  __shared__ int fail_sm;
+  const PanelJob job{n, lda, k0, n, n, xr, chunks, (int)blockIdx.x, nullptr, 0};
+  panel_step(job, A, Ldiag, info, cp_smem, dinv, &fail_sm, threadIdx.x, nullptr, nullptr);
+}
+
+template <int KS>
+__device__ __forceinline__ void update_tile(int n, int lda, int k0, int ri, int rj, bool diag,
+                                            const double* __restrict__ A, double* As, double* Bs, int tid, int bar,
+                                            double (&c)[2][2][4]) {
+  constexpr int LDS = KS + 4;
+  auto sync = [bar] {
+    if (bar == 0) __syncthreads();
+    else group_sync(bar);
+  };
+  const int lane = tid & 31, warp = tid >> 5;
+  const double* bs = diag ? As : Bs;
+  const int wm = warp / 4, wn = warp % 4;
+  const int g = lane >> 2, q = lane & 3;
+#pragma unroll
+  for (int i = 0; i < 2; ++i)
+#pragma unroll
+    for (int j = 0; j < 2; ++j) c[i][j][0] = c[i][j][1] = c[i][j][2] = c[i][j][3] = 0.0;
+  const double* arow = As + (wm * 32 + g) * LDS + q;
+  const double* brow = bs + (wn * 16 + g) * LDS + q;
+#pragma unroll 1
+  for (int ks = 0; ks < CB; ks += KS) {
+    if (ks) sync();
+    for (int e = tid; e < 2 * CT * (KS / 4); e += C_THREADS) {
+      const int row = e / (KS / 4), ch = (e % (KS / 4)) * 4;
+      const bool isA = row < CT;
+      if (!isA && diag) continue;
+      const int grow = isA ? ri + row : rj + (row - CT);
+      double* dst = (isA ? As + row * LDS : Bs + (row - CT) * LDS) + ch;
+      if (grow < n) {
+        const double* src = A + (size_t)grow * lda + k0 + ks + ch;
         cp_async16(dst, src);
         cp_async16(dst + 2, src + 2);
       } else {
@@ -439,139 +643,44 @@
       }
     }
     cp_async_commit();
-  }
-  {
-    const int g = lane >> 2, q = lane & 3;
-    const int nrow16 = (xr + 15) / 16;
-    double c[2][2][4];
-#pragma unroll
-    for (int i = 0; i < 2; ++i)
-#pragma unroll
-      for (int j = 0; j < 2; ++j) c[i][j][0] = c[i][j][1] = c[i][j][2] = c[i][j][3] = 0.0;
-#pragma unroll
-    for (int half = 0; half < 2; ++half) {
-      if (half == 0) cp_async_wait<1>();
-      else cp_async_wait<0>();
-      __syncthreads();
+    cp_async_wait<0>();
+    sync();
 #pragma unroll 2
-      for (int kk = half * 64; kk < half * 64 + 64; kk += 16) {
-        double a[2][8], b[2][4];
-#pragma unroll
-        for (int j = 0; j < 2; ++j)
-#pragma unroll
-          for (int e = 0; e < 4; ++e) b[j][e] = Ls[(warp * 16 + j * 8 + g) * CLD + kk + q + 4 * e];
-#pragma unroll
-        for (int i = 0; i < 2; ++i) {
-          if (i < nrow16) {
-#pragma unroll
-            for (int e = 0; e < 8; ++e) {
-              const int r = i * 16 + g + 8 * (e & 1);
-              a[i][e] = r < xr ? Ts[r * CLD + kk + q + 4 * (e >> 1)] : 0.0;
-            }
-#pragma unroll
-            for (int j = 0; j < 2; ++j) dmma_m16n8k16(c[i][j], a[i], b[j]);
-          }
-        }
-      }
-    }
-#pragma unroll
-    for (int i = 0; i < 2; ++i) {
-#pragma unroll
-      for (int h = 0; h < 2; ++h) {
-        const int rr = i * 16 + g + 8 * h;
-        if (i >= nrow16 || rr >= nrows) continue;
-        const int r = r0 + rr;
-#pragma unroll
-        for (int j = 0; j < 2; ++j) {
-          const int col = t0 + warp * 16 + j * 8 + 2 * q;
-          double* p = A + (size_t)r * lda + col;
-          if (col <= r) atomicAdd(p, -c[i][j][2 * h]);
-          if (col + 1 <= r) atomicAdd(p + 1, -c[i][j][2 * h + 1]);
-        }
-      }
+    for (int kk = 0; kk < KS; kk += 16) {
+      double a[2][8], b[2][4];
+#pragma unroll
+      for (int i = 0; i < 2; ++i)
+#pragma unroll
+        for (int e = 0; e < 8; ++e) a[i][e] = arow[(i * 16 + 8 * (e & 1)) * LDS + kk + 4 * (e >> 1)];
+#pragma unroll
+      for (int j = 0; j < 2; ++j)
+#pragma unroll
+        for (int e = 0; e < 4; ++e) b[j][e] = brow[j * 8 * LDS + kk + 4 * e];
+#pragma unroll
+      for (int i = 0; i < 2; ++i)
+#pragma unroll
+        for (int j = 0; j < 2; ++j) dmma_m16n8k16(c[i][j], a[i], b[j]);
     }
   }
 }
 
 constexpr int CUD = 68;
-enum { CU_ALL = 0, CU_NEXT = 1, CU_REST = 2 };
-__global__ void __launch_bounds__(C_THREADS, 2) chol_update_kernel(int n, int lda, int k0, int t0, int mode,
-                                                                    double* __restrict__ A, int band_end, int arrow_lo,
-                                                                    int all_red) {
+__global__ void __launch_bounds__(C_THREADS, 2) chol_update_kernel(int n, int lda, int k0, int t0,
+                                                                    double* __restrict__ A) {
   extern __shared__ __align__(16) double cu_smem[];
   double* As = cu_smem;
   double* Bs = cu_smem + CT * CUD;
-  int bi, bj;
-  {
-    const int t = blockIdx.x;
-    if (mode == CU_NEXT) {
-      const int T = (max(0, min(band_end, n) - t0) + 63) / 64 + (band_end >= n ? 0 : (n - arrow_lo + 63) / 64);
-      if (t < T - 2) { bi = 2 + t; bj = 2; }
-      else { bi = 3 + (t - (T - 2)); bj = 3; }
-    } else {
-      bi = (int)((sqrtf(8.0f * (float)t + 1.0f) - 1.0f) * 0.5f);
-      while ((bi + 1) * (bi + 2) / 2 <= t) ++bi;
-      while (bi * (bi + 1) / 2 > t) --bi;
-      bj = t - bi * (bi + 1) / 2;
-      const int skip = mode == CU_REST ? 4 : 0;
-      bi += skip;
-      bj += skip;
-    }
-  }
-  const bool diag = bi == bj;
+  const int t = blockIdx.x;
+  int bi = (int)((sqrtf(8.0f * (float)t + 1.0f) - 1.0f) * 0.5f);
+  while ((bi + 1) * (bi + 2) / 2 <= t) ++bi;
+  while (bi * (bi + 1) / 2 > t) --bi;
+  const int bj = t - bi * (bi + 1) / 2;
   const int tid = threadIdx.x, lane = tid & 31, warp = tid >> 5;
-  const int T1v = band_end >= n ? (1 << 30) : (band_end - t0) / 64;
-  auto vrow = [&](int v) { return v < T1v ? t0 + v * 64 : arrow_lo + (v - T1v) * 64; };
-  const int ri = vrow(bi), rj = vrow(bj);
-  const double* bs = diag ? As : Bs;
+  const int ri = t0 + bi * CT, rj = t0 + bj * CT;
+  double c[2][2][4];
+  update_tile<64>(n, lda, k0, ri, rj, bi == bj, A, As, Bs, tid, 0, c);
   const int wm = warp / 4, wn = warp % 4;
   const int g = lane >> 2, q = lane & 3;
-  double c[2][2][4];
-#pragma unroll
-  for (int i = 0; i < 2; ++i)
-#pragma unroll
-    for (int j = 0; j < 2; ++j) c[i][j][0] = c[i][j][1] = c[i][j][2] = c[i][j][3] = 0.0;
-  const double* arow = As + (wm * 32 + g) * CUD + q;
-  const double* brow = bs + (wn * 16 + g) * CUD + q;
-#pragma unroll 1
-  for (int half = 0; half < 2; ++half) {
-    if (half) __syncthreads();
-    for (int e = tid; e < 2 * CT * 16; e += C_THREADS) {
-      const int row = e >> 4, ch = (e & 15) * 4;
-      const bool isA = row < CT;
-      if (!isA && diag) continue;
-      const int grow = isA ? ri + row : rj + (row - CT);
-      double* dst = (isA ? As + row * CUD : Bs + (row - CT) * CUD) + ch;
-      if (grow < n) {
-        const double* src = A + (size_t)grow * lda + k0 + half * 64 + ch;
-        cp_async16(dst, src);
-        cp_async16(dst + 2, src + 2);
-      } else {
-        *reinterpret_cast<double2*>(dst) = make_double2(0.0, 0.0);
-        *reinterpret_cast<double2*>(dst + 2) = make_double2(0.0, 0.0);
-      }
-    }
-    cp_async_commit();
-    cp_async_wait<0>();
-    __syncthreads();
-#pragma unroll 2
-    for (int kk = 0; kk < 64; kk += 16) {
-      double a[2][8], b[2][4];
-#pragma unroll
-      for (int i = 0; i < 2; ++i)
-#pragma unroll
-        for (int e = 0; e < 8; ++e) a[i][e] = arow[(i * 16 + 8 * (e & 1)) * CUD + kk + 4 * (e >> 1)];
-#pragma unroll
-      for (int j = 0; j < 2; ++j)
-#pragma unroll
-        for (int e = 0; e < 4; ++e) b[j][e] = brow[j * 8 * CUD + kk + 4 * e];
-#pragma unroll
-      for (int i = 0; i < 2; ++i)
-#pragma unroll
-        for (int j = 0; j < 2; ++j) dmma_m16n8k16(c[i][j], a[i], b[j]);
-    }
-  }
-  const bool red = all_red || mode == CU_NEXT || (mode == CU_REST && bj < 6);
 #pragma unroll
   for (int i = 0; i < 2; ++i) {
 #pragma unroll
@@ -584,10 +693,7 @@
         if (col > r) continue;
         double* p = A + (size_t)r * lda + col;
         const double v0 = c[i][j][2 * h], v1 = c[i][j][2 * h + 1];
-        if (red) {
-          atomicAdd(p, -v0);
-          if (col + 1 <= r) atomicAdd(p + 1, -v1);
-        } else if (col + 1 <= r) {
+        if (col + 1 <= r) {
           double2 v = *reinterpret_cast<double2*>(p);
           v.x -= v0;
           v.y -= v1;
@@ -600,37 +706,117 @@
   }
 }
 
+constexpr int CP_THREADS = 2 * C_THREADS;
+__global__ void __launch_bounds__(CP_THREADS, 1) chol_persistent_kernel(const __grid_constant__ CholArgs a) {
+  extern __shared__ __align__(16) double cp_smem[];
+  __shared__ double dinv[CB];
+  __shared__ int fail_sm, ticket_sm[2];
+  const int tid = threadIdx.x;
+  int* const step_ctr = a.ctr + 1;
+  int* const col_ctr = a.ctr + 1 + a.nblk;
+  int* const chunk_flag = a.ctr + 1 + 2 * a.nblk;
+  if ((int)blockIdx.x < a.panel_ctas) {
+    if (tid >= C_THREADS) return;
+    StepGeo gp{};
+    for (int b = 0; b < a.nblk; ++b) {
+      const StepGeo g = step_geo(a, b);
+      for (int v = blockIdx.x; v <= g.chunks; v += a.panel_ctas) {
+        long long* stamp = a.stamps && v == min(1, g.chunks) ? a.stamps + 4 * b : nullptr;
+        if (stamp && tid == 0) stamp[0] = globaltimer();
+        int need = 0;
+        if (tid < 32 && b > 0) {
+          for (int s = tid; s + 2 <= b; s += 32) need += step_tiles_in_col(step_geo(a, s), a.n, b);
+          need = __reduce_add_sync(0xffffffffu, need);
+        }
+        if (tid == 0 && b > 0) {
+          const int band_hi = min(g.band_end, a.n), c1r = (max(0, band_hi - (g.k0 + CB)) + g.xr - 1) / g.xr;
+          const int r0 = v < 1 ? 0 : v - 1 < c1r ? g.k0 + CB + (v - 1) * g.xr : g.arrow_lo + (v - 1 - c1r) * g.xr;
+          const int r1 = v < 1 ? 0 : min(r0 + g.xr, v - 1 < c1r ? band_hi : a.n);
+          for (int part = 0; part < 2; ++part) {
+            int r = part ? r0 : g.k0;
+            const int rend = part ? r1 : min(g.k0 + CB, a.n);
+            while (r < rend) {
+              int next;
+              const int c = step_chunk_at(gp, a.n, r, &next);
+              if (c) chol_wait(chunk_flag + c, 0, -1, b, a.info, false);
+              r = next;
+            }
+          }
+          if (need) chol_wait(col_ctr + b, 0, -1, need, a.info, false);
+        }
+        panel_sync();
+        const PanelJob job{a.n, a.lda, g.k0, g.band_end, g.arrow_lo, g.xr, g.chunks, v, b ? step_ctr + b - 1 : nullptr, gp.chunks};
+        panel_step(job, a.A, a.Ldiag, a.info, cp_smem, dinv, &fail_sm, tid, b + 1 < a.nblk ? step_ctr + b : nullptr, stamp);
+        panel_sync();
+        if (tid == 0 && v > 0) asm volatile("st.release.gpu.global.s32 [%0], %1;" ::"l"(chunk_flag + v), "r"(b + 1) : "memory");
+      }
+      gp = g;
+    }
+    return;
+  }
+  const int grp = tid / C_THREADS, u = tid % C_THREADS, bar = 1 + grp;
+  double* As = cp_smem + grp * 2 * CT * CUD;
+  double* Bs = As + CT * CUD;
+  int s = 0, base = 0, ready = -1;
+  StepGeo g = step_geo(a, 0);
+  int ntile = step_tiles(g);
+  for (;;) {
+    if (u == 0) ticket_sm[grp] = atomicAdd(a.ctr, 1);
+    group_sync(bar);
+    const int t = ticket_sm[grp];
+    group_sync(bar);
+    while (t >= base + ntile && s + 1 < a.nblk) {
+      base += ntile;
+      g = step_geo(a, ++s);
+      ntile = s + 1 < a.nblk ? step_tiles(g) : 0;
+    }
+    if (t >= base + ntile) break;
+    int lt = t - base, bj = 2;
+    while (lt >= g.T - bj) {
+      lt -= g.T - bj;
+      ++bj;
+    }
+    const int bi = bj + lt;
+    if (s != ready) {
+      if (u == 0) chol_wait(step_ctr + s, 0, 0xffff, g.chunks, a.info, true);
+      group_sync(bar);
+      ready = s;
+    }
+    const int ri = tile_row(g, bi), rj = tile_row(g, bj);
+    double c[2][2][4];
+    update_tile<64>(a.n, a.lda, g.k0, ri, rj, bi == bj, a.A, As, Bs, u, bar, c);
+    const int lane = u & 31, warp = u >> 5, wm = warp / 4, wn = warp % 4, gq = lane >> 2, q = lane & 3;
+#pragma unroll
+    for (int i = 0; i < 2; ++i) {
+#pragma unroll
+      for (int h = 0; h < 2; ++h) {
+        const int r = ri + wm * 32 + i * 16 + gq + 8 * h;
+        if (r >= a.n) continue;
+#pragma unroll
+        for (int j = 0; j < 2; ++j) {
+          const int col = rj + wn * 16 + j * 8 + 2 * q;
+          if (col > r) continue;
+          double* p = a.A + (size_t)r * a.lda + col;
+          atomicAdd(p, -c[i][j][2 * h]);
+          if (col + 1 <= r) atomicAdd(p + 1, -c[i][j][2 * h + 1]);
+        }
+      }
+    }
+    __threadfence();
+    group_sync(bar);
+    if (u == 0) {
+      __threadfence();
+      atomicAdd(col_ctr + rj / CB, 1);
+    }
+  }
+}
 
 size_t chol_workspace_doubles(int n) {
   const int nblk = (n + CB - 1) / CB;
-  return (size_t)nblk * CB * CB + (size_t)(nblk + 1) / 2 + 1;
+  return (size_t)nblk * CB * CB;
 }
 
 namespace {
-
-struct CholStreams {
-  cudaStream_t side_lo = nullptr, side_mid = nullptr, cap = nullptr;
-  cudaEvent_t ev_col = nullptr, ev_upd[2] = {nullptr, nullptr}, ev_bulk[3] = {nullptr, nullptr, nullptr};
-  bool ready = false;
-};
-
-int chol_streams(CholStreams** out) {
-  static thread_local CholStreams s;
-  if (!s.ready) {
-    int lo = 0, hi = 0;
-    VGG_CUDA_CHECK(cudaDeviceGetStreamPriorityRange(&lo, &hi));
-    VGG_CUDA_CHECK(cudaStreamCreateWithPriority(&s.side_lo, cudaStreamNonBlocking, lo));
-    VGG_CUDA_CHECK(cudaStreamCreateWithPriority(&s.side_mid, cudaStreamNonBlocking, (lo + hi) / 2));
-    VGG_CUDA_CHECK(cudaStreamCreateWithPriority(&s.cap, cudaStreamNonBlocking, hi));
-    VGG_CUDA_CHECK(cudaEventCreateWithFlags(&s.ev_col, cudaEventDisableTiming));
-    VGG_CUDA_CHECK(cudaEventCreateWithFlags(&s.ev_upd[0], cudaEventDisableTiming));
-    VGG_CUDA_CHECK(cudaEventCreateWithFlags(&s.ev_upd[1], cudaEventDisableTiming));
-    for (int i = 0; i < 3; ++i) VGG_CUDA_CHECK(cudaEventCreateWithFlags(&s.ev_bulk[i], cudaEventDisableTiming));
-    s.ready = true;
-  }
-  *out = &s;
-  return VGG_OK;
-}
 
 int chol_sms() {
   static const int v = [] {
@@ -642,6 +828,9 @@
   return v;
 }
 
+constexpr size_t CP_SMEM = sizeof(double) * (CB + C_RPC_MAX) * CLD;
+static_assert(2 * 2 * CT * CUD <= (CB + C_RPC_MAX) * CLD, "update groups exceed the panel CTA's shared memory");
+
 int chol_set_attrs() {
   static bool done = false;
   if (done) return VGG_OK;
@@ -649,95 +838,35 @@
                                       (int)(sizeof(double) * (CB + C_RPC_MAX) * CLD)));
   VGG_CUDA_CHECK(cudaFuncSetAttribute(chol_update_kernel, cudaFuncAttributeMaxDynamicSharedMemorySize,
                                       (int)(sizeof(double) * 2 * CT * CUD)));
+  VGG_CUDA_CHECK(cudaFuncSetAttribute(chol_persistent_kernel, cudaFuncAttributeMaxDynamicSharedMemorySize,
+                                      (int)CP_SMEM));
   done = true;
   return VGG_OK;
 }
 
-int chol_panel_rows(int below1, int below2, int* chunks) {
-  const int sms = chol_sms();
-  int xr = C_RPC;
-  for (;; xr += 4) {
-    *chunks = (below1 + xr - 1) / xr + (below2 + xr - 1) / xr;
-    if (1 + *chunks <= sms || xr >= C_RPC_MAX) return xr;
-  }
-}
-
-int chol_enqueue(int n, int lda, double* A, double* Ldiag, int* info, int* flags, const std::vector<int>& end_blk,
-                 int arrow_blk, cudaStream_t st, CholStreams* cs, bool lookahead) {
+int chol_program_order(int n, int lda, double* A, double* Ldiag, int* info, cudaStream_t st) {
   const int nblk = (n + CB - 1) / CB;
-  const size_t smem_u = sizeof(double) * 2 * CT * CUD;
-  const bool banded = lookahead && (int)end_blk.size() >= nblk && arrow_blk > 0;
-  auto band_rows = [&](int b, int* band_end, int* arrow_lo) {
-    if (!banded) {
-      *band_end = *arrow_lo = n;
-      return;
-    }
-    *band_end = std::min(n, end_blk[b] * CB);
-    *arrow_lo = std::min(n, std::max(arrow_blk * CB, *band_end));
-    if (*band_end >= n || *arrow_lo <= *band_end) *band_end = *arrow_lo = n;
-  };
-  auto panel = [&](int b) -> int {
-    const int k0 = b * CB;
-    int band_end, arrow_lo, chunks;
-    band_rows(b, &band_end, &arrow_lo);
-    const int below1 = std::max(0, std::min(band_end, n) - (k0 + CB));
-    const int below2 = band_end >= n ? 0 : n - arrow_lo;
-    const int xr = chol_panel_rows(below1, below2, &chunks);
-    const size_t smem_p = sizeof(double) * (CB + xr) * CLD;
-    const int fuse = lookahead ? 1 : 0;
-    chol_panel_kernel<<<1 + chunks, C_THREADS, smem_p, st>>>(n, lda, k0, A, Ldiag, info, flags, fuse, band_end, arrow_lo, xr);
+  CholArgs a;
+  a.n = n;
+  a.sms = chol_sms();
+  a.banded = 0;
+  a.xr_fixed = 0;
+  for (int b = 0; b < nblk; ++b) {
+    const StepGeo g = step_geo(a, b);
+    if (b > 0) {
+      const int T = (n - g.k0 + CT - 1) / CT;
+      chol_update_kernel<<<T * (T + 1) / 2, C_THREADS, sizeof(double) * 2 * CT * CUD, st>>>(n, lda, g.k0 - CB, g.k0, A);
+      VGG_LAUNCH_CHECK();
+    }
+    chol_panel_kernel<<<1 + g.chunks, C_THREADS, sizeof(double) * (CB + g.xr) * CLD, st>>>(n, lda, g.k0, A, Ldiag, info,
+                                                                                            g.xr, g.chunks);
     VGG_LAUNCH_CHECK();
-    return VGG_OK;
-  };
-  int rc;
-  if ((rc = panel(0))) return rc;
-  if (!lookahead) {
-    for (int b = 0; b + 1 < nblk; ++b) {
-      const int k0 = b * CB, t0 = k0 + CB;
-      const int T = (n - t0 + CT - 1) / CT;
-      chol_update_kernel<<<T * (T + 1) / 2, C_THREADS, smem_u, st>>>(n, lda, k0, t0, CU_ALL, A, n, n, 0);
-      VGG_LAUNCH_CHECK();
-      if ((rc = panel(b + 1))) return rc;
-    }
-    return VGG_OK;
-  }
-  bool have_u1[2] = {false, false}, have_u2[3] = {false, false, false};
-  for (int b = 0; b + 1 < nblk; ++b) {
-    const int k0 = b * CB, t0 = k0 + CB;
-    int band_end, arrow_lo;
-    band_rows(b, &band_end, &arrow_lo);
-    const int T = (std::max(0, std::min(band_end, n) - t0) + CT - 1) / CT + (band_end >= n ? 0 : (n - arrow_lo + CT - 1) / CT);
-    const int all_red = band_end >= n ? 0 : 1;
-    const int n_u1 = T > 2 ? (T - 2) + (T > 3 ? T - 3 : 0) : 0;
-    const int n_u2 = T > 4 ? (T - 4) * (T - 3) / 2 : 0;
-    have_u1[b & 1] = false;
-    have_u2[b % 3] = false;
-    if (n_u1 > 0) {
-      VGG_CUDA_CHECK(cudaEventRecord(cs->ev_col, st));
-      VGG_CUDA_CHECK(cudaStreamWaitEvent(cs->side_mid, cs->ev_col, 0));
-      if (b >= 2 && have_u2[(b - 2) % 3]) VGG_CUDA_CHECK(cudaStreamWaitEvent(cs->side_mid, cs->ev_bulk[(b - 2) % 3], 0));
-      chol_update_kernel<<<n_u1, C_THREADS, smem_u, cs->side_mid>>>(n, lda, k0, t0, CU_NEXT, A, band_end, arrow_lo, all_red);
-      VGG_LAUNCH_CHECK();
-      VGG_CUDA_CHECK(cudaEventRecord(cs->ev_upd[b & 1], cs->side_mid));
-      have_u1[b & 1] = true;
-      if (n_u2 > 0) {
-        VGG_CUDA_CHECK(cudaStreamWaitEvent(cs->side_lo, cs->ev_col, 0));
-        chol_update_kernel<<<n_u2, C_THREADS, smem_u, cs->side_lo>>>(n, lda, k0, t0, CU_REST, A, band_end, arrow_lo, all_red);
-        VGG_LAUNCH_CHECK();
-        VGG_CUDA_CHECK(cudaEventRecord(cs->ev_bulk[b % 3], cs->side_lo));
-        have_u2[b % 3] = true;
-      }
-    }
-    if (b >= 1 && have_u1[(b - 1) & 1]) VGG_CUDA_CHECK(cudaStreamWaitEvent(st, cs->ev_upd[(b - 1) & 1], 0));
-    if (b >= 2 && have_u2[(b - 2) % 3]) VGG_CUDA_CHECK(cudaStreamWaitEvent(st, cs->ev_bulk[(b - 2) % 3], 0));
-    if ((rc = panel(b + 1))) return rc;
-  }
-  for (int i = 0; i < 2; ++i)
-    if (have_u1[i]) VGG_CUDA_CHECK(cudaStreamWaitEvent(st, cs->ev_upd[i], 0));
-  for (int i = 0; i < 3; ++i)
-    if (have_u2[i]) VGG_CUDA_CHECK(cudaStreamWaitEvent(st, cs->ev_bulk[i], 0));
+  }
   return VGG_OK;
 }
+
+long long* g_chol_stamps = nullptr;
+int g_chol_stamped_blocks = 0;
 
 }
 
@@ -747,46 +876,64 @@
   int rc;
   if ((rc = chol_set_attrs())) return rc;
   VGG_CUDA_CHECK(cudaMemsetAsync(info, 0, sizeof(int), st));
-  const int nblk0 = (n + CB - 1) / CB;
-  int* flags = reinterpret_cast<int*>(Ldiag + (size_t)nblk0 * CB * CB);
-  VGG_CUDA_CHECK(cudaMemsetAsync(flags, 0, sizeof(int) * (size_t)nblk0, st));
-  static const bool use_graph = [] { const char* e = getenv("VGG_CHOL_GRAPH"); return !(e && e[0] == '0'); }();
   const int nblk = (n + CB - 1) / CB;
-  CholStreams* cs = nullptr;
-  if ((rc = chol_streams(&cs))) return rc;
-  if (nblk < 3 || !use_graph) return chol_enqueue(n, lda, A, Ldiag, info, flags, end_blk, arrow_blk, st, cs, nblk >= 3);
-  typedef std::tuple<double*, int, int, int*, double*, unsigned long long> Key;
-  static thread_local std::map<Key, cudaGraphExec_t> cache;
-  unsigned long long band_hash = (unsigned long long)arrow_blk;
-  for (int v : end_blk) band_hash = band_hash * 1000003ull + (unsigned long long)(v + 1);
-  const Key key(A, n, lda, info, Ldiag, band_hash);
-  auto it = cache.find(key);
-  if (it == cache.end()) {
-    const long long launches_before = g_launch_count;
-    cudaGraph_t graph = nullptr;
-    VGG_CUDA_CHECK(cudaStreamBeginCapture(cs->cap, cudaStreamCaptureModeThreadLocal));
-    rc = chol_enqueue(n, lda, A, Ldiag, info, flags, end_blk, arrow_blk, cs->cap, cs, true);
-    const cudaError_t ce = cudaStreamEndCapture(cs->cap, &graph);
-    g_launch_count = launches_before;
-    if (rc) {
-      if (graph) cudaGraphDestroy(graph);
-      return rc;
-    }
-    VGG_CUDA_CHECK(ce);
-    cudaGraphExec_t exec = nullptr;
-    VGG_CUDA_CHECK(cudaGraphInstantiate(&exec, graph, 0));
-    cudaGraphDestroy(graph);
-    if (cache.size() > 8) {
-      for (auto& kv : cache) cudaGraphExecDestroy(kv.second);
-      cache.clear();
-    }
-    it = cache.emplace(key, exec).first;
-  }
-  VGG_CUDA_CHECK(cudaGraphLaunch(it->second, st));
-  g_launch_count += 1 + 3 * (nblk - 1);
+  if (nblk < 3) return chol_program_order(n, lda, A, Ldiag, info, st);
+  CholArgs a;
+  a.n = n;
+  a.lda = lda;
+  a.nblk = nblk;
+  a.arrow_blk = arrow_blk;
+  a.sms = chol_sms();
+  a.banded = (int)end_blk.size() >= nblk && arrow_blk > 0;
+  VGG_REQUIRE(!a.banded || nblk <= CHOL_MAX_BLK, "banded Cholesky: too many blocks");
+  for (int b = 0; b < CHOL_MAX_BLK; ++b) a.end_blk[b] = (unsigned short)(a.banded && b < nblk ? end_blk[b] : 0);
+  a.xr_fixed = C_RPC_MAX;
+  a.panel_ctas = 1;
+  for (int b = 0; b < nblk; ++b) a.panel_ctas = std::max(a.panel_ctas, 1 + step_geo(a, b).chunks);
+  a.panel_ctas = std::min(a.panel_ctas, a.sms - a.sms / 4);
+  a.A = A;
+  a.Ldiag = Ldiag;
+  a.info = info;
+  a.ctr = reinterpret_cast<int*>(Ldiag + (size_t)(nblk - 1) * CB * CB);
+  a.stamps = g_chol_stamps && nblk <= CHOL_MAX_BLK ? g_chol_stamps : nullptr;
+  g_chol_stamped_blocks = a.stamps ? nblk : 0;
+  int max_chunks = 0;
+  for (int b = 0; b < nblk; ++b) max_chunks = std::max(max_chunks, step_geo(a, b).chunks);
+  const size_t nctr = 2 + 2 * (size_t)nblk + max_chunks;
+  VGG_REQUIRE(nctr * sizeof(int) <= sizeof(double) * CB * CB, "Cholesky order too large for the step counters");
+  VGG_CUDA_CHECK(cudaMemsetAsync(a.ctr, 0, sizeof(int) * nctr, st));
+  void* args[] = {&a};
+  VGG_CUDA_CHECK(cudaLaunchCooperativeKernel((const void*)chol_persistent_kernel, dim3(a.sms), dim3(CP_THREADS), args,
+                                             CP_SMEM, st));
+  VGG_LAUNCH_CHECK();
   return VGG_OK;
 }
 
+}
+
+extern "C" int vgg_dev_chol_stamps(int enable) {
+  using namespace vgg;
+  if (enable && !g_chol_stamps) VGG_CUDA_CHECK(cudaMalloc(&g_chol_stamps, sizeof(long long) * 4 * CHOL_MAX_BLK));
+  if (!enable && g_chol_stamps) {
+    VGG_CUDA_CHECK(cudaDeviceSynchronize());
+    VGG_CUDA_CHECK(cudaFree(g_chol_stamps));
+    g_chol_stamps = nullptr;
+  }
+  return VGG_OK;
+}
+
+extern "C" int vgg_dev_chol_last_stamps(long long* stamps_host, int cap_steps, int* nblk) {
+  using namespace vgg;
+  VGG_REQUIRE(nblk && (stamps_host || cap_steps <= 0), "chol stamps: bad arguments");
+  *nblk = g_chol_stamped_blocks;
+  if (!g_chol_stamps || g_chol_stamped_blocks == 0) {
+    *nblk = 0;
+    return VGG_OK;
+  }
+  VGG_CUDA_CHECK(cudaDeviceSynchronize());
+  const int m = std::min(cap_steps, g_chol_stamped_blocks);
+  if (m > 0) VGG_CUDA_CHECK(cudaMemcpy(stamps_host, g_chol_stamps, sizeof(long long) * 4 * m, cudaMemcpyDeviceToHost));
+  return VGG_OK;
 }
 
 extern "C" int vgg_dev_chol128_probe(int reps, const double* A_host, double* L_host, long long* prof13_host) {
diff --git a/vggsfm_b200/csrc/dev_probes.h b/vggsfm_b200/csrc/dev_probes.h
--- a/vggsfm_b200/csrc/dev_probes.h
+++ b/vggsfm_b200/csrc/dev_probes.h
@@ -5,6 +5,8 @@
 int vgg_dev_blocks_timing(int enable);
 int vgg_dev_blocks_last_ms(double* ms);
 int vgg_dev_chol128_probe(int reps, const double* A_host, double* L_host, long long* prof13_host);
+int vgg_dev_chol_stamps(int enable);
+int vgg_dev_chol_last_stamps(long long* stamps_host, int cap_steps, int* nblk);
 int vgg_dev_syrk_f64(int Kpad, int Dpad, const double* Zt, double* Cmat, void* stream);
 int vgg_dev_syrk_f64_band(int Kpad, int Dpad, const double* Zt, double* Cmat, void* stream, const int* ranges_host,
                           int count);
```

After: 347.6, median of 6. 2.7% higher.
